# Deci-AI/super-gradients

Measured on NVIDIA H100. Metric: images/sec YOLO-NAS-S 640 bf16 train, higher is better.
Workload: dtype bf16

## Files before the change

### include/sgb200.h

```cpp
#ifndef SGB200_H_
#define SGB200_H_

#include <stdint.h>

#ifdef __cplusplus
extern "C" {
#endif

#define SGB_OK 0
#define SGB_E_INVALID (-1)
#define SGB_E_UNSUPPORTED (-2)
#define SGB_E_CUDA (-3)
#define SGB_E_ARCH (-4)

#define SGB_ACT_NONE 0
#define SGB_ACT_RELU 1
#define SGB_ACT_SILU 2

typedef uint16_t sgb_bf16;

typedef struct SgbConvDesc {
  int32_t N, H, W, C;
  int32_t K, R, S;
  int32_t P, Q;
  int32_t stride, pad;
  int32_t x_pitch, x_off;
  int32_t y_pitch, y_off;
  int32_t up2;
  int32_t centre_from;
} SgbConvDesc;

typedef struct SgbEpilogue {
  const float* scale;
  const float* shift;
  const sgb_bf16* residual;
  double* stats;
  int32_t stats_repl;
  int32_t act;
  int32_t out_f32;
} SgbEpilogue;

const char* sgb_last_error(void);
int sgb_version(void);
int sgb_check_device(void);
int64_t sgb_sm100_launches(void);
int64_t sgb_conv_halo_launches(void);
void sgb_conv_force_im2col(int on);
int64_t sgb_conv_wgrad_halo_launches(void);
void sgb_conv_wgrad_force_im2col(int on);

int sgb_conv_fprop(const SgbConvDesc* d, const sgb_bf16* x, const sgb_bf16* w_krsc, void* y, const SgbEpilogue* ep,
                   void* stream);
int sgb_conv_dgrad(const SgbConvDesc* d, const sgb_bf16* dy, const sgb_bf16* w_crsk, sgb_bf16* dx, int accumulate,
                   void* stream);
int sgb_conv_wgrad(const SgbConvDesc* d, const sgb_bf16* x, const sgb_bf16* dy, float* dw_krsc, void* stream);
int sgb_weight_prepare(const float* w_oihw, int K, int C, int R, int S, int c_pad, sgb_bf16* w_krsc, sgb_bf16* w_crsk,
                       const float* scale, int add_identity, void* stream);
int sgb_wgrad_to_oihw(const float* dw_krsc, int K, int C, int R, int S, int c_pad, float* g_oihw, int accumulate,
                      void* stream);
typedef struct SgbWeightItem {
  const float* w;
  const float* scale;
  sgb_bf16* krsc;
  sgb_bf16* crsk;
  int32_t K, C, R, S, c_pad, add_identity;
  int32_t kp, koff, etaps, etap;
  int64_t start;
} SgbWeightItem;
typedef struct SgbWgradItem {
  const float* dw;
  float* g;
  int32_t K, C, R, S, c_pad, accumulate;
  int64_t start;
} SgbWgradItem;
int sgb_weight_prepare_batch(const SgbWeightItem* items_dev, int n_items, int64_t total, void* stream);
typedef struct SgbAlphaItem {
  const float* dw1;
  const float* w1;
  const float* alpha;
  const float* dab;
  const float* bias1;
  float* g_w1;
  float* g_bias;
  float* g_alpha;
  int32_t K, C, c_pad, pad_;
} SgbAlphaItem;
int sgb_qarep_alpha_finish_batch(const SgbAlphaItem* items_dev, int n_items, void* stream);
int sgb_wgrad_to_oihw_batch(const SgbWgradItem* items_dev, int n_items, int64_t total, void* stream);
int sgb_convt2x2_fprop(const SgbConvDesc* d, const sgb_bf16* x_small, const sgb_bf16* w_up, const float* bias,
                       sgb_bf16* y_up, void* stream);

int sgb_nchw_f32_to_nhwc_bf16(const float* x, int N, int C, int H, int W, sgb_bf16* y, int y_pitch, int y_off, int c_out,
                              void* stream);
int sgb_stem_patches_f32(const float* x, int N, int C, int H, int W, int R, int stride, int pad, sgb_bf16* y, int P, int Q, int c_out,
                         void* stream);
int sgb_nhwc_bf16_to_nchw_f32(const sgb_bf16* x, int N, int C, int H, int W, int x_pitch, int x_off, float* y,
                              void* stream);

typedef struct SgbBnDesc {
  int64_t M;
  int32_t C;
  int32_t x_pitch, x_off;
  int32_t y_pitch, y_off;
  int32_t r_pitch, r_off;
  float eps, momentum;
  int32_t act;
  int32_t stats_repl;
  int32_t dy_pitch, dy_off;
  int64_t hw;
  const float* sample_scale;
  int32_t dy2_split, dy2_pitch, dy2_off, dy2_reserved;
  const void* dy2;
  const double* count;
  float param_scale;
  int32_t count_reserved;
} SgbBnDesc;
int sgb_bn_act_fwd(const SgbBnDesc* d, const sgb_bf16* x, const double* stats, const float* gamma, const float* beta,
                   float* running_mean, float* running_var, const sgb_bf16* residual, sgb_bf16* y, float* save_mean,
                   float* save_rstd, void* stream);
int sgb_bn_act_infer(const SgbBnDesc* d, const sgb_bf16* x, const float* gamma, const float* beta,
                     const float* running_mean, const float* running_var, const sgb_bf16* residual, sgb_bf16* y,
                     void* stream);
int sgb_bn_act_bwd_reduce(const SgbBnDesc* d, const sgb_bf16* dy, const sgb_bf16* x, const sgb_bf16* y, const float* gamma,
                          const float* beta, const float* save_mean, const float* save_rstd, double* sums, void* stream);
int sgb_bn_act_bwd_apply(const SgbBnDesc* d, const sgb_bf16* dy, const sgb_bf16* x, const sgb_bf16* y,
                         const float* gamma, const float* beta, const float* save_mean, const float* save_rstd,
                         const double* sums, sgb_bf16* dx, sgb_bf16* dresidual, float* dgamma, float* dbeta, void* stream);
int sgb_channel_stats(const sgb_bf16* x, int64_t M, int C, int pitch, int off, double* stats, void* stream);

typedef struct SgbQarepDesc {
  int64_t M;
  int32_t C;
  int32_t pitch3, off3, pitchu, offu, pitcho, offo;
  float eps3, eps_post, momentum;
  int32_t act;
  int32_t use_post_bn;
  int32_t pitchd, offd;
  int32_t pitchr, offr;
  const void* res;
  const float* res_alpha;
  const double* count;
  float param_scale;
  int32_t count_reserved;
} SgbQarepDesc;
int sgb_qarep_moments(const SgbQarepDesc* d, const sgb_bf16* y3, const sgb_bf16* u, double* moments, void* stream);
int sgb_qarep_fwd(const SgbQarepDesc* d, const sgb_bf16* y3, const sgb_bf16* u, const double* moments,
                  const float* gamma3, const float* beta3, const float* bias1_alpha, const float* gamma_p,
                  const float* beta_p, float* rm3, float* rv3, float* rm_p, float* rv_p, sgb_bf16* out, float* coef,
                  void* stream);
int sgb_qarep_fwd_fused(const SgbQarepDesc* d, const sgb_bf16* y3, const sgb_bf16* u, double* moments, const float* gamma3,
                        const float* beta3, const float* bias1_alpha, const float* gamma_p, const float* beta_p, float* rm3, float* rv3,
                        float* rm_p, float* rv_p, sgb_bf16* out, float* coef, void* stream);
int sgb_qarep_bwd_reduce(const SgbQarepDesc* d, const sgb_bf16* dout, const sgb_bf16* out, const sgb_bf16* y3,
                         const sgb_bf16* u, const float* coef, double* sums, void* stream);
int sgb_qarep_bwd_apply(const SgbQarepDesc* d, const sgb_bf16* dout, const sgb_bf16* out, const sgb_bf16* y3,
                        const sgb_bf16* u, const float* coef, const double* sums, const float* gamma3,
                        const float* gamma_p, sgb_bf16* dy3, sgb_bf16* du, float* dgamma3, float* dbeta3,
                        float* dbias1a, float* dgamma_p, float* dbeta_p, void* stream);
int sgb_bn_act_bwd_fused(const SgbBnDesc* d, const sgb_bf16* dy, const sgb_bf16* x, const sgb_bf16* y, const float* gamma,
                         const float* beta, const float* save_mean, const float* save_rstd, double* sums, sgb_bf16* dx,
                         sgb_bf16* dresidual, float* dgamma, float* dbeta, void* stream);
int sgb_bn_act_fwd_fused(const SgbBnDesc* d, const sgb_bf16* x, double* stats, const float* gamma, const float* beta,
                         float* running_mean, float* running_var, const sgb_bf16* residual, sgb_bf16* y, float* save_mean,
                         float* save_rstd, void* stream);
int sgb_qarep_bwd_fused(const SgbQarepDesc* d, const sgb_bf16* dout, const sgb_bf16* y3, const sgb_bf16* u, const float* coef,
                        double* sums, const float* gamma3, const float* gamma_p, sgb_bf16* dy3, sgb_bf16* du, float* dgamma3,
                        float* dbeta3, float* dbias1a, float* dgamma_p, float* dbeta_p, void* stream);

int sgb_stem_gemm(const SgbQarepDesc* d, const sgb_bf16* xp, const sgb_bf16* w, sgb_bf16* y, void* stream);
int sgb_stem_qarep_moments(const SgbQarepDesc* d, const sgb_bf16* xp, const sgb_bf16* w, double* moments, void* stream);
int sgb_stem_qarep_fwd(const SgbQarepDesc* d, const sgb_bf16* xp, const sgb_bf16* w, const double* moments, const float* gamma3,
                       const float* beta3, const float* bias1_alpha, const float* gamma_p, const float* beta_p, float* rm3, float* rv3,
                       float* rm_p, float* rv_p, sgb_bf16* out, float* coef, void* stream);
int sgb_stem_qarep_bwd_reduce(const SgbQarepDesc* d, const sgb_bf16* dout, const sgb_bf16* xp, const sgb_bf16* w, const float* coef,
                              double* sums, void* stream);
int sgb_stem_qarep_bwd_apply(const SgbQarepDesc* d, const sgb_bf16* dout, const sgb_bf16* xp, const sgb_bf16* w, const float* coef,
                             const double* sums, const float* gamma3, const float* gamma_p, sgb_bf16* dy3, sgb_bf16* du, float* dgamma3,
                             float* dbeta3, float* dbias1a, float* dgamma_p, float* dbeta_p, void* stream);
int64_t sgb_stem_recompute_launches(void);


int sgb_maxpool_fwd(const sgb_bf16* x, int N, int H, int W, int C, int x_pitch, int x_off, int k, int stride, int pad,
                    sgb_bf16* y, int P, int Q, int y_pitch, int y_off, uint8_t* idx, void* stream);
int sgb_maxpool_bwd(const sgb_bf16* dy, int N, int H, int W, int C, int k, int stride, int pad, int P, int Q,
                    int dy_pitch, int dy_off, const uint8_t* idx, float* dx_f32, void* stream);
int sgb_maxpool_bwd_bf16(const sgb_bf16* dy, int N, int H, int W, int C, int k, int stride, int pad, int P, int Q,
                         int dy_pitch, int dy_off, const uint8_t* idx, sgb_bf16* dx, int dx_pitch, void* stream);
int sgb_axpby(const sgb_bf16* x1, int p1, int o1, float a, const sgb_bf16* x2, int p2, int o2, float b, sgb_bf16* y,
              int py, int oy, int64_t M, int C, void* stream);
int sgb_scale_add(const sgb_bf16* x1, int p1, int o1, const float* a_dev, const sgb_bf16* x2, int p2, int o2, sgb_bf16* y,
                  int py, int oy, int64_t M, int C, void* stream);
int sgb_scale_add_dot(const sgb_bf16* x1, int p1, int o1, const float* a_dev, const sgb_bf16* x2, int p2, int o2, const sgb_bf16* xd, int pd,
                      int od, sgb_bf16* y, int py, int oy, int64_t M, int C, double* out_dot, void* stream);
int sgb_channel_dot(const sgb_bf16* a, int pa, int oa, const sgb_bf16* b, int pb, int ob, int64_t M, int C, double* out,
                    void* stream);
int sgb_f32_to_bf16(const float* x, sgb_bf16* y, int64_t n, void* stream);
int sgb_avgpool_fwd(const sgb_bf16* x, int N, int HW, int C, sgb_bf16* y, void* stream);
int sgb_avgpool_bwd(const sgb_bf16* dy, int N, int HW, int C, sgb_bf16* dx, void* stream);

int sgb_dfl_decode(const sgb_bf16* reg, int reg_pitch, const sgb_bf16* cls, int cls_pitch, int N, int Hf, int Wf,
                   int L, int anchor_base, int ncls, int reg_max, float stride, float cell_offset, float* pred_bboxes,
                   float* pred_scores, float* cls_logits, float* reg_distri, void* stream);

int sgb_pose_keypoint_decode(const sgb_bf16* pose, int pose_pitch, const sgb_bf16* logit, int logit_pitch, int logit_off, int N,
                             int Hf, int Wf, int L, int anchor_base, int J, float stride, float cell_offset,
                             float offset_multiplier, int compensate_grid_cell_offset, float* pose_coords, float* pose_scores,
                             float* pose_logits, void* stream);

typedef struct SgbLossDesc {
  int32_t B, L, ncls, reg_max;
  int32_t n_max;
  int32_t topk;
  float alpha, beta;
  float w_cls, w_iou, w_dfl;
  int32_t iou_type;
} SgbLossDesc;
int sgb_tal_assign(const SgbLossDesc* d, const float* cls_logits, const float* reg_distri, const float* anchor_points,
                   const float* stride_tensor, const float* gt_boxes, const int32_t* gt_labels, const uint8_t* gt_valid,
                   int32_t* assigned_label, float* assigned_box, float* assigned_score, double* sums, void* workspace,
                   int64_t workspace_bytes, void* stream);
int64_t sgb_tal_workspace_bytes(const SgbLossDesc* d);
int sgb_atss_assign(const SgbLossDesc* d, const float* reg_distri, const float* anchors, const float* anchor_points,
                    const float* stride_tensor, const int32_t* level_sizes, int32_t n_levels, const float* gt_boxes,
                    const int32_t* gt_labels, const uint8_t* gt_valid, int32_t* assigned_label, float* assigned_box,
                    float* assigned_score, double* sums, void* workspace, int64_t workspace_bytes, void* stream);
int64_t sgb_atss_workspace_bytes(const SgbLossDesc* d);
int sgb_dfl_iou_loss_fwd_bwd(const SgbLossDesc* d, const float* cls_logits, const float* reg_distri,
                             const float* anchor_points, const float* stride_tensor, const int32_t* assigned_label,
                             const float* assigned_box, const float* assigned_score, double* sums, float grad_scale,
                             float* grad_cls, float* grad_reg, void* stream);
int sgb_focal_cls_fwd_bwd(const SgbLossDesc* d, const float* cls_logits, const int32_t* assigned_label,
                          const float* assigned_score, double* sums, float grad_scale, float alpha, float* grad_cls,
                          void* stream);
int sgb_loss_finalize(const SgbLossDesc* d, const double* sums, float* loss_out, void* stream);
int sgb_head_grad_scatter(const float* grad, int gC, int N, int HW, int L, int anchor_base, sgb_bf16* dy, int pitch,
                          void* stream);

typedef struct SgbPoseLossDesc {
  int32_t B, L, J, reg_max;
  int32_t n_max;
  int32_t topk;
  float alpha, beta;
  float w_cls, w_iou, w_dfl, w_pose_cls, w_pose_reg;
  int32_t iou_type;
  int32_t cls_type;
  int32_t pose_cls_type;
  int32_t multiply_by_oks;
  int32_t rescale_with_score;
} SgbPoseLossDesc;
int64_t sgb_pose_tal_workspace_bytes(const SgbPoseLossDesc* d);
int sgb_pose_tal_assign(const SgbPoseLossDesc* d, const float* cls_logits, const float* reg_distri, const float* pose_coords,
                        const float* anchor_points, const float* stride_tensor, const float* gt_boxes, const float* gt_poses,
                        const uint8_t* gt_crowd, const uint8_t* gt_valid, const float* sigmas, int32_t* assigned_gt,
                        float* assigned_score, double* sums, void* workspace, int64_t workspace_bytes, void* stream);
int sgb_pose_loss_fwd_bwd(const SgbPoseLossDesc* d, const float* cls_logits, const float* reg_distri, const float* pose_coords,
                          const float* pose_logits, const float* anchor_points, const float* stride_tensor,
                          const float* gt_boxes, const float* gt_poses, const float* sigmas, const int32_t* assigned_gt,
                          const float* assigned_score, double* sums, float grad_scale, float* grad_cls, float* grad_reg,
                          float* grad_pose, float* grad_pose_logits, void* stream);
int sgb_pose_loss_finalize(const SgbPoseLossDesc* d, const double* sums, float* loss_out, void* stream);

typedef struct SgbNmsDesc {
  int32_t B, L, ncls;
  float score_thr;
  double iou_thr;
  int32_t top_k, max_out;
  int32_t multi_label;
  int32_t class_agnostic;
  int32_t thr_inclusive;
} SgbNmsDesc;
int64_t sgb_nms_workspace_bytes(const SgbNmsDesc* d);
int sgb_batched_nms(const SgbNmsDesc* d, const float* boxes, const float* scores, float* out, int32_t* out_idx,
                    int32_t* out_count, void* workspace, int64_t workspace_bytes, void* stream);

int sgb_sliding_window_gather(const sgb_bf16* canvas, int32_t B, int32_t H, int32_t W, int32_t pitch, const int32_t* tiles_host,
                              const int32_t* tiles, int32_t T, int32_t tile, sgb_bf16* out, void* stream);
int64_t sgb_sliding_window_merge_workspace_bytes(int32_t B, const int32_t* image_tiles_host, int32_t T, int32_t P, int32_t ncls);
int sgb_sliding_window_merge(const float* rows, const int32_t* counts, const int32_t* tiles, const int32_t* image_tiles_host,
                             const int32_t* image_tiles, int32_t B, int32_t T, int32_t P, int32_t ncls, double iou_thr, float* out,
                             int32_t* out_count, void* workspace, int64_t workspace_bytes, void* stream);
int32_t sgb_sliding_window_merge_launches(int32_t B, const int32_t* image_tiles_host, int32_t T, int32_t P);

#define SGB_MATCH_MAX_THRESHOLDS 32
typedef struct SgbMatchDesc {
  int32_t B;
  int32_t max_preds;
  int32_t max_targets;
  int32_t max_crowd;
  int32_t n_thresholds;
  int32_t top_k;
  int32_t denormalize_targets;
  float height, width;
} SgbMatchDesc;
int sgb_detection_matching(const SgbMatchDesc* d, const float* preds, const int32_t* pred_count, const float* targets,
                           const int32_t* target_count, const float* crowd, const int32_t* crowd_count, const float* thresholds,
                           uint8_t* matched, uint8_t* ignore, void* stream);

#define SGB_DISTANCE_EUCLIDEAN 0
#define SGB_DISTANCE_MANHATTAN 1
int sgb_detection_distance_matching(const SgbMatchDesc* d, int32_t metric, const float* preds, const int32_t* pred_count,
                                    const float* targets, const int32_t* target_count, const float* crowd,
                                    const int32_t* crowd_count, const float* thresholds, uint8_t* matched, uint8_t* ignore,
                                    void* stream);

int sgb_pose_keypoint_matching(const float* poses, const float* scores, const int32_t* pred_count, const float* gt_joints,
                               const float* gt_boxes, const float* gt_areas, const uint8_t* gt_flags, const int32_t* gt_count,
                               const float* sigmas, const float* thresholds, int32_t B, int32_t max_preds, int32_t max_targets,
                               int32_t n_joints, int32_t n_thresholds, int32_t top_k, uint8_t* matched, uint8_t* ignore,
                               float* used_scores, int32_t* used_count, int32_t* n_targets, float* oks_out, void* stream);

typedef struct SgbPreprocDesc {
  int32_t src_h, src_w, src_c;
  int32_t src_pitch;
  int32_t dst_h, dst_w;
  int32_t out_h, out_w;
  int32_t pad_top, pad_left;
  int32_t out_pitch;
  int32_t reverse_channels;
  int32_t normalize;
  float pad_value;
  double max_value;
  float mean[4], std[4];
} SgbPreprocDesc;
int sgb_preprocess_u8(const SgbPreprocDesc* d, const uint8_t* src, sgb_bf16* out, void* stream);

#define SGB_RS_OFFSET 0
#define SGB_RS_H 1
#define SGB_RS_W 2
#define SGB_RS_PITCH 3
#define SGB_RS_RESIZED_H 4
#define SGB_RS_RESIZED_W 5
#define SGB_RS_CROP_TOP 6
#define SGB_RS_CROP_LEFT 7
#define SGB_RS_FIELDS 8
int sgb_resample_crop_u8(const int64_t* table_host, const int64_t* table, const uint8_t* src, int64_t src_bytes, int32_t batch,
                         int32_t channels, int32_t out_h, int32_t out_w, int32_t out_pitch, int32_t reverse_channels,
                         double max_value, const float* mean_host, const float* std_host, sgb_bf16* out, void* stream);

#define SGB_AUG_OFFSET 0
#define SGB_AUG_H 1
#define SGB_AUG_W 2
#define SGB_AUG_AFFINE 3
#define SGB_AUG_AFF_H 4
#define SGB_AUG_AFF_W 5
#define SGB_AUG_M 6
#define SGB_AUG_AFF_BORDER 12
#define SGB_AUG_SWAP 13
#define SGB_AUG_HSV 14
#define SGB_AUG_DH 15
#define SGB_AUG_DS 16
#define SGB_AUG_DV 17
#define SGB_AUG_BGR 18
#define SGB_AUG_FLIP 19
#define SGB_AUG_MIX 20
#define SGB_AUG_MIX_OFFSET 21
#define SGB_AUG_MIX_H 22
#define SGB_AUG_MIX_W 23
#define SGB_AUG_MIX_FLIP 24
#define SGB_AUG_MIX_R1_H 25
#define SGB_AUG_MIX_R1_W 26
#define SGB_AUG_MIX_CANVAS_H 27
#define SGB_AUG_MIX_CANVAS_W 28
#define SGB_AUG_MIX_BORDER 29
#define SGB_AUG_MIX_R2_H 30
#define SGB_AUG_MIX_R2_W 31
#define SGB_AUG_MIX_X 32
#define SGB_AUG_MIX_Y 33
#define SGB_AUG_RS_H 34
#define SGB_AUG_RS_W 35
#define SGB_AUG_MOS 36
#define SGB_AUG_MOS_CANVAS_H 37
#define SGB_AUG_MOS_CANVAS_W 38
#define SGB_AUG_MOS_XC 39
#define SGB_AUG_MOS_YC 40
#define SGB_AUG_MOS_BORDER 41
#define SGB_AUG_MOS_TILE 42
#define SGB_AUG_MOS_TILES 4
#define SGB_AUG_T_OFFSET 0
#define SGB_AUG_T_H 1
#define SGB_AUG_T_W 2
#define SGB_AUG_T_RH 3
#define SGB_AUG_T_RW 4
#define SGB_AUG_T_X1 5
#define SGB_AUG_T_Y1 6
#define SGB_AUG_T_X2 7
#define SGB_AUG_T_Y2 8
#define SGB_AUG_T_SX 9
#define SGB_AUG_T_SY 10
#define SGB_AUG_MOS_TILE_FIELDS 11
#define SGB_AUG_FIELDS 86
int sgb_detection_augment(const int64_t* table_host, const int64_t* table, const uint8_t* src, int64_t src_bytes, int32_t batch,
                          int32_t channels, int32_t out_h, int32_t out_w, int32_t out_pitch, int32_t pad_value, double max_value,
                          int32_t hsv_simd_block, sgb_bf16* out, void* stream);

#define SGB_IN_OFFSET 0
#define SGB_IN_H 1
#define SGB_IN_W 2
#define SGB_IN_FILTER 3
#define SGB_IN_FLIP 4
#define SGB_IN_WS_OFFSET 5
#define SGB_IN_OP 6
#define SGB_IN_OP_FIELDS 7
#define SGB_IN_OPS 2
#define SGB_IN_FIELDS 20
#define SGB_IN_OP_NONE 0
#define SGB_IN_OP_AFFINE 1
#define SGB_IN_OP_INVERT 2
#define SGB_IN_OP_POSTERIZE 3
#define SGB_IN_OP_SOLARIZE 4
#define SGB_IN_OP_SOLARIZE_ADD 5
#define SGB_IN_OP_BRIGHTNESS 6
#define SGB_IN_OP_CONTRAST 7
#define SGB_IN_OP_AUTOCONTRAST 8
#define SGB_IN_OP_EQUALIZE 9
#define SGB_IN_OP_COLOR 10
#define SGB_IN_OP_SHARPNESS 11
int sgb_imagenet_augment(const int64_t* table_host, const int64_t* table, const uint8_t* src, int64_t src_bytes, uint8_t* workspace,
                         int64_t workspace_bytes, int32_t batch, int32_t size, int32_t out_pitch, const int32_t* fill_host,
                         const float* mean_host, const float* std_host, int32_t mix_mode, float lam, float one_minus_lam,
                         const int32_t* box_host, sgb_bf16* out, void* stream);

#define SGB_CF_SOURCE 0
#define SGB_CF_TOP 1
#define SGB_CF_LEFT 2
#define SGB_CF_FLIP 3
#define SGB_CF_FIELDS 4
#define SGB_CF_SIZE 32
#define SGB_CF_PAD 4
int sgb_cifar_augment(const int32_t* table_host, const int32_t* table, const uint8_t* src, int64_t src_images, int32_t batch,
                      int32_t out_pitch, const float* mean_host, const float* std_host, sgb_bf16* out, void* stream);

#define SGB_POSE_NSUB 0
#define SGB_POSE_CANVAS_H 1
#define SGB_POSE_CANVAS_W 2
#define SGB_POSE_MOSAIC_PAD 3
#define SGB_POSE_RS_H 4
#define SGB_POSE_RS_W 5
#define SGB_POSE_PAD_TOP 6
#define SGB_POSE_PAD_LEFT 7
#define SGB_POSE_PAD_VALUE 8
#define SGB_POSE_SUB 16
#define SGB_POSE_SUB_FIELDS 32
#define SGB_POSE_FIELDS 144
#define SGB_POSE_S_OFFSET 0
#define SGB_POSE_S_H 1
#define SGB_POSE_S_W 2
#define SGB_POSE_S_FLIP 3
#define SGB_POSE_S_BC 4
#define SGB_POSE_S_MEAN 5
#define SGB_POSE_S_CONTRAST 8
#define SGB_POSE_S_BRIGHTNESS 9
#define SGB_POSE_S_REVERSE 10
#define SGB_POSE_S_HSV 11
#define SGB_POSE_S_DH 12
#define SGB_POSE_S_DS 13
#define SGB_POSE_S_DV 14
#define SGB_POSE_S_ROT 15
#define SGB_POSE_S_AFFINE 16
#define SGB_POSE_S_M 17
#define SGB_POSE_S_MODE 23
#define SGB_POSE_S_BORDER 24
#define SGB_POSE_S_WS_OFFSET 25
#define SGB_POSE_S_Y 26
#define SGB_POSE_S_X 27
#define SGB_POSE_S_RH 28
#define SGB_POSE_S_RW 29
int sgb_pose_augment(const int64_t* table_host, const int64_t* table, const uint8_t* src, int64_t src_bytes, uint8_t* workspace,
                     int64_t workspace_bytes, int32_t batch, int32_t out_size, int32_t out_pitch, double max_value, int32_t hsv_simd_block,
                     sgb_bf16* out, void* stream);

int sgb_classify_rows(const void* logits, int64_t N, int32_t C, int64_t row_stride, int32_t logits_bf16, const int64_t* target,
                      const void* soft_target, int64_t target_stride, int32_t target_bf16, int32_t k, int64_t* counters,
                      int32_t* label, float* confidence, void* stream);

int sgb_sgd_step(float* p, const float* g, float* mom, int64_t n, const float* hp, void* stream);
int sgb_adamw_step(float* p, const float* g, float* m, float* v, int64_t n, const float* hp, void* stream);
int sgb_adam_step(float* p, const float* g, float* m, float* v, int64_t n, const float* hp, void* stream);
int sgb_rmsprop_step(float* p, const float* g, float* square_avg, float* momentum_buffer, float* grad_avg, int64_t n, const float* hp, void* stream);
int sgb_rmsprop_tf_step(float* p, const float* g, float* square_avg, float* momentum_buffer, float* grad_avg, int64_t n, const float* hp, void* stream);
int sgb_lion_step(float* p, const float* g, float* m, int64_t n, const float* hp, void* stream);
int sgb_lamb_grad_sqnorm(const float* g, const int64_t* chunks, int32_t nchunk, const float* hp, double* partials, void* stream);
int sgb_lamb_step(float* p, const float* g, float* m, float* v, float* update, int64_t n_decay, const int64_t* chunks, int32_t nchunk,
                  const float* hp, double* partials, void* stream);
int sgb_clip_grad_norm(const float* g, const int64_t* chunks, int32_t nchunk, float* hp, int32_t hp_len, int32_t gs_col, float max_norm, double* partials,
                       float* norm_coef, void* stream);
int sgb_ema_update(float* ema, const float* p, int64_t n, const float* decay, void* stream);

#define SGB_AVG_MAX_SLOTS 64
int sgb_average_snapshots(const float* const* slots, int32_t k, int64_t n, float* out, void* stream);

#ifdef __cplusplus
}
#endif
#endif
```

### super_gradients_b200/csrc/capi.cu

```cuda
#include <cstdarg>
#include <cstdio>

#include "common.cuh"
#include "conv_sm100.h"

static thread_local char g_err[512] = "";

void sgb_set_error(const char* fmt, ...) {
  va_list ap;
  va_start(ap, fmt);
  vsnprintf(g_err, sizeof(g_err), fmt, ap);
  va_end(ap);
}

int sgb_cuda_check(cudaError_t e, const char* what) {
  if (e == cudaSuccess) return SGB_OK;
  sgb_set_error("%s: %s", what, cudaGetErrorString(e));
  return SGB_E_CUDA;
}

extern "C" const char* sgb_last_error(void) { return g_err; }
extern "C" int sgb_version(void) { return 100; }
extern "C" int sgb_check_device(void) {
  int dev = 0;
  if (int rc = sgb_cuda_check(cudaGetDevice(&dev), "cudaGetDevice")) return rc;
  cudaDeviceProp prop;
  if (int rc = sgb_cuda_check(cudaGetDeviceProperties(&prop, dev), "cudaGetDeviceProperties")) return rc;
  if (prop.major != 9) {
    sgb_set_error("libsgb200 is built for sm_90a only; device is sm_%d%d", prop.major, prop.minor);
    return SGB_E_ARCH;
  }
  return SGB_OK;
}

extern "C" int64_t sgb_sm100_launches(void) { return (int64_t)sm100::launch_count(); }
extern "C" int64_t sgb_conv_halo_launches(void) { return (int64_t)sm100::halo_launch_count(); }
extern "C" void sgb_conv_force_im2col(int on) { sm100::force_im2col(on != 0); }
extern "C" int64_t sgb_conv_wgrad_halo_launches(void) { return (int64_t)sm100::wgrad_halo_launch_count(); }
extern "C" void sgb_conv_wgrad_force_im2col(int on) { sm100::wgrad_force_im2col(on != 0); }
```

### super_gradients_b200/csrc/conv_sm100.cu

```cuda
#include <cuda.h>

#include <cstdio>
#include <cstdlib>
#include <cstring>

#include "common.cuh"
#include "conv_sm100.h"
#include "sm100_host.h"
#include "sm100_ptx.cuh"

namespace sm100 {

constexpr int BLOCK_M = 128;
constexpr int NUM_THREADS = 384;
constexpr int CONSUMER_THREADS = 256;
constexpr int MAX_STAGES = 8;

struct Params {
  int M;
  int N;
  int C;
  int KC;
  int n_tiles;
  int stages;
  int P, Q;
  int stride, pad;
  int b_cols_per_tap;
  int ntaps;
  signed char tap_dh[9], tap_dw[9], tap_b[9];
  int out_mode, o_mul, oh_add, ow_add, outH, outW;
  int halo_tw, halo_thw;
  long long y_pitch;
  int y_off;
  bf16* y;
  const float* scale;
  const float* shift;
  const bf16* residual;
  double* stats;
  int stats_repl;
  int act;
  int centre_n, centre_c;
};

template <int BN>
__device__ __forceinline__ int off_centre_steps(const Params& p, int nt, int steps, int step_ch) {
  if (p.centre_n > 0 && nt * BN >= p.centre_n) return 0;
  if (p.centre_c > 0) return (p.centre_c + step_ch - 1) / step_ch;
  return steps;
}
constexpr int CENTRE_TAP = 4;

__device__ __forceinline__ long long out_row(const Params& p, long long m) {
  if (p.out_mode == 0) return m;
  const int pq = p.P * p.Q;
  const int n = (int)(m / pq);
  const int rem = (int)(m - (long long)n * pq);
  const int j = rem / p.Q, i = rem - j * p.Q;
  return ((long long)n * p.outH + j * p.o_mul + p.oh_add) * p.outW + i * p.o_mul + p.ow_add;
}

__device__ __forceinline__ void consumer_sync() { asm volatile("bar.sync 1, %0;" ::"n"(CONSUMER_THREADS) : "memory"); }
template <int WARPS>
__device__ __forceinline__ void group_sync(int wg) {
  if (WARPS == 8)
    consumer_sync();
  else
    asm volatile("bar.sync %0, 128;" ::"r"(2 + wg) : "memory");
}

constexpr uint32_t CTRL_BAR_BYTES = 16u * MAX_STAGES;

template <int BN, int WARPS = 8>
__device__ __forceinline__ void tile_epilogue(const Params& p, const float (&acc)[BN / 2], const long long (&orow)[2],
                                              const bool (&row_ok)[2], int nt, int wg, int wq, int lane, float* s_part,
                                              float* s_stats) {
  const int n0 = nt * BN;
  const int ncols = min(BN, p.N - n0);
  bf16* yrow[2];
  const bf16* rrow[2];
#pragma unroll
  for (int h = 0; h < 2; ++h) {
    yrow[h] = p.y + orow[h] * p.y_pitch + p.y_off + n0;
    rrow[h] = p.residual ? p.residual + orow[h] * p.y_pitch + p.y_off + n0 : nullptr;
  }
#pragma unroll
  for (int j = 0; j < BN / 8; ++j) {
    const int col = 8 * j + 2 * (lane & 3);
    const bool col_ok = col < ncols;
    float sum0 = 0.f, sum1 = 0.f, sq0 = 0.f, sq1 = 0.f;
#pragma unroll
    for (int h = 0; h < 2; ++h) {
      float v0 = acc[4 * j + 2 * h], v1 = acc[4 * j + 2 * h + 1];
      const bool ok = row_ok[h] && col_ok;
      if (p.scale && col_ok) {
        v0 *= p.scale[n0 + col];
        v1 *= p.scale[n0 + col + 1];
      }
      if (p.shift && col_ok) {
        v0 += p.shift[n0 + col];
        v1 += p.shift[n0 + col + 1];
      }
      if (rrow[h] && ok) {
        const uint32_t rr = *reinterpret_cast<const uint32_t*>(rrow[h] + col);
        v0 += __uint_as_float(rr << 16);
        v1 += __uint_as_float(rr & 0xffff0000u);
      }
      if (p.act != SGB_ACT_NONE) {
        v0 = apply_act(v0, p.act);
        v1 = apply_act(v1, p.act);
      }
      __nv_bfloat162 hh = __floats2bfloat162_rn(v0, v1);
      const uint32_t pk = *reinterpret_cast<uint32_t*>(&hh);
      if (ok) {
        *reinterpret_cast<uint32_t*>(yrow[h] + col) = pk;
        const float lo = __uint_as_float(pk << 16), hi = __uint_as_float(pk & 0xffff0000u);
        sum0 += lo;
        sum1 += hi;
        sq0 = fmaf(lo, lo, sq0);
        sq1 = fmaf(hi, hi, sq1);
      }
    }
    if (p.stats) {
#pragma unroll
      for (int o = 4; o < 32; o <<= 1) {
        sum0 += __shfl_xor_sync(0xffffffffu, sum0, o);
        sum1 += __shfl_xor_sync(0xffffffffu, sum1, o);
        sq0 += __shfl_xor_sync(0xffffffffu, sq0, o);
        sq1 += __shfl_xor_sync(0xffffffffu, sq1, o);
      }
      if (lane < 4) {
        float* part = s_part + (WARPS == 8 ? wg * 4 + wq : wq) * 2 * BN;
        part[col] = sum0;
        part[col + 1] = sum1;
        part[BN + col] = sq0;
        part[BN + col + 1] = sq1;
      }
    }
  }
  if (p.stats) {
    group_sync<WARPS>(wg);
    for (int i = threadIdx.x - 128 - (WARPS == 8 ? 0 : 128 * wg); i < 2 * BN; i += WARPS * 32) {
      const int which = i / BN, c = i - which * BN;
      if (c < ncols) {
        float v = 0.f;
#pragma unroll
        for (int w = 0; w < WARPS; ++w) v += s_part[w * 2 * BN + i];
        s_stats[which * p.N + n0 + c] += v;
      }
    }
    group_sync<WARPS>(wg);
  }
}

__device__ __forceinline__ void flush_stats(const Params& p, const float* s_stats) {
  if (p.stats) {
    double* st = p.stats + (long long)(blockIdx.x & (p.stats_repl - 1)) * 2 * p.N;
    for (int i = threadIdx.x; i < 2 * p.N; i += NUM_THREADS) {
      const float v = s_stats[i];
      if (v != 0.f) atomicAdd(&st[i], (double)v);
    }
  }
}

template <int BN, bool SKIP>
__global__ void __launch_bounds__(NUM_THREADS, 1)
conv_wgmma_kernel(const __grid_constant__ CUtensorMap map_a, const __grid_constant__ CUtensorMap map_b, const Params p) {
  extern __shared__ __align__(1024) unsigned char smem_raw[];
  const uint32_t smem_base = (smem_u32(smem_raw) + 1023u) & ~1023u;
  const uint32_t a_bytes = BLOCK_M * p.KC * 2, b_bytes = BN * p.KC * 2;
  const uint32_t stage_bytes = a_bytes + ((b_bytes + 1023u) & ~1023u);
  const uint32_t ctrl = smem_base + p.stages * stage_bytes;
  auto full_bar = [&](int s) { return ctrl + 8u * s; };
  auto empty_bar = [&](int s) { return ctrl + 8u * (MAX_STAGES + s); };
  float* s_part = reinterpret_cast<float*>(smem_raw + (ctrl + CTRL_BAR_BYTES - smem_u32(smem_raw)));
  float* s_stats = s_part + 8 * 2 * BN;

  const int warp = threadIdx.x >> 5, lane = threadIdx.x & 31;
  const int m_tiles = (p.M + BLOCK_M - 1) / BLOCK_M;
  const int total_tiles = m_tiles * p.n_tiles;
  const int chunks = (p.C + p.KC - 1) / p.KC;

  if (threadIdx.x == 0) {
    for (int s = 0; s < p.stages; ++s) {
      mbar_init(full_bar(s), 1);
      mbar_init(empty_bar(s), 8);
    }
    asm volatile("fence.mbarrier_init.release.cluster;" ::: "memory");
    asm volatile("fence.proxy.async.shared::cta;" ::: "memory");
  }
  if (p.stats)
    for (int i = threadIdx.x; i < 2 * p.N; i += NUM_THREADS) s_stats[i] = 0.f;
  __syncthreads();

  if (warp == 0) {
    if (elect_one()) {
      int stg = 0;
      uint32_t par = 1;
      const int pq = p.P * p.Q;
      for (int tile = blockIdx.x; tile < total_tiles; tile += gridDim.x) {
        const int mt = tile / p.n_tiles, nt = tile - mt * p.n_tiles;
        const int m0 = mt * BLOCK_M;
        const int n_img = m0 / pq;
        const int rem = m0 - n_img * pq;
        const int p0 = rem / p.Q, q0 = rem - p0 * p.Q;
        const int w0 = q0 * p.stride - p.pad, h0 = p0 * p.stride - p.pad;
        const int off = SKIP ? off_centre_steps<BN>(p, nt, chunks, p.KC) : chunks;
        for (int tap = 0; tap < p.ntaps; ++tap) {
          const int r = p.tap_dh[tap], s = p.tap_dw[tap];
          const int btap = p.tap_b[tap];
          const int n_ck = tap == CENTRE_TAP ? chunks : off;
          for (int ck = 0; ck < n_ck; ++ck) {
            mbar_wait(empty_bar(stg), par);
            const uint32_t sa = smem_base + stg * stage_bytes, sb = sa + a_bytes;
            mbar_expect_tx(full_bar(stg), a_bytes + b_bytes);
            tma_load_im2col_4d(sa, &map_a, full_bar(stg), ck * p.KC, w0, h0, n_img, (uint16_t)s, (uint16_t)r);
            tma_load_2d(sb, &map_b, full_bar(stg), btap * p.b_cols_per_tap + ck * p.KC, nt * BN);
            if (++stg == p.stages) {
              stg = 0;
              par ^= 1;
            }
          }
        }
      }
    }
  } else if (warp >= 4) {
    const int wg = (warp >> 2) - 1;
    const int wq = warp & 3;
    const int row_bytes = p.KC * 2;
    const uint32_t sbo = 8u * (uint32_t)row_bytes;
    const int ksteps = p.KC / 16;
    float acc[BN / 2];
    int stg = 0;
    uint32_t par = 0;
    for (int tile = blockIdx.x; tile < total_tiles; tile += gridDim.x) {
      const int mt = tile / p.n_tiles, nt = tile - mt * p.n_tiles;
      const int k_iters = SKIP ? 8 * off_centre_steps<BN>(p, nt, chunks, p.KC) + chunks : p.ntaps * chunks;
      int prev = -1;
      for (int k = 0; k < k_iters; ++k) {
        mbar_wait(full_bar(stg), par);
        const uint32_t sa = smem_base + stg * stage_bytes, sb = sa + a_bytes;
        const uint32_t sa_wg = sa + (uint32_t)wg * 64u * (uint32_t)row_bytes;
        wgmma_fence();
        for (int j = 0; j < ksteps; ++j) {
          const uint64_t da = smem_desc(sa_wg + 32u * j, row_bytes, 16u, sbo), db = smem_desc(sb + 32u * j, row_bytes, 16u, sbo);
          mma_kk<BN>(acc, da, db, (k | j) != 0);
        }
        wgmma_commit();
        if (prev >= 0) {
          wgmma_wait<1>();
          __syncwarp();
          if (lane == 0) mbar_arrive(empty_bar(prev));
        }
        prev = stg;
        if (++stg == p.stages) {
          stg = 0;
          par ^= 1;
        }
      }
      wgmma_wait<0>();
      fence_regs(acc);
      __syncwarp();
      if (lane == 0 && prev >= 0) mbar_arrive(empty_bar(prev));

      const long long m_lo = (long long)mt * BLOCK_M + wg * 64 + wq * 16 + (lane >> 2);
      long long orow[2];
      bool row_ok[2];
#pragma unroll
      for (int h = 0; h < 2; ++h) {
        const long long m = m_lo + 8 * h;
        row_ok[h] = m < p.M;
        orow[h] = out_row(p, row_ok[h] ? m : 0);
      }
      tile_epilogue<BN>(p, acc, orow, row_ok, nt, wg, wq, lane, s_part, s_stats);
    }
  }
  __syncthreads();
  flush_stats(p, s_stats);
}

constexpr int HALO_W = 10, HALO_H = 10, HALO_TILE = 8;
constexpr uint32_t HALO_CG_BYTES = 1664;
constexpr uint32_t HALO_CTRL_BYTES = CTRL_BAR_BYTES + 16;
constexpr int HALO_MAX_STAGES = 6;

template <int BN, bool SKIP>
__global__ void __launch_bounds__(NUM_THREADS, BN <= 48 ? 2 : 1)
conv3x3_halo_kernel(const __grid_constant__ CUtensorMap map_a, const __grid_constant__ CUtensorMap map_b, const Params p) {
  extern __shared__ __align__(1024) unsigned char smem_raw[];
  const uint32_t smem_base = (smem_u32(smem_raw) + 1023u) & ~1023u;
  const int ksteps = p.C / 16;
  constexpr uint32_t b_box = BN * 32;
  const uint32_t b_bytes = 9u * ksteps * b_box;
  const uint32_t a_stage = ((uint32_t)(p.C / 8) * HALO_CG_BYTES + 1023u) & ~1023u;
  const uint32_t sb = smem_base, sa0 = smem_base + ((b_bytes + 1023u) & ~1023u);
  const uint32_t ctrl = sa0 + p.stages * a_stage;
  auto full_bar = [&](int s) { return ctrl + 8u * s; };
  auto empty_bar = [&](int s) { return ctrl + 8u * (MAX_STAGES + s); };
  const uint32_t b_bar = ctrl + CTRL_BAR_BYTES;
  float* s_part = reinterpret_cast<float*>(smem_raw + (ctrl + HALO_CTRL_BYTES - smem_u32(smem_raw)));
  float* s_stats = s_part + 8 * 2 * BN;

  const int warp = threadIdx.x >> 5, lane = threadIdx.x & 31;
  const int m_tiles = p.M;
  const int nt = blockIdx.x % p.n_tiles;
  const int mt_step = gridDim.x / p.n_tiles;
  const int mt0 = blockIdx.x / p.n_tiles;
  const int off = SKIP ? off_centre_steps<BN>(p, nt, ksteps, 16) : ksteps;

  if (threadIdx.x == 0) {
    for (int s = 0; s < p.stages; ++s) {
      mbar_init(full_bar(s), 1);
      mbar_init(empty_bar(s), 4);
    }
    mbar_init(b_bar, 1);
    asm volatile("fence.mbarrier_init.release.cluster;" ::: "memory");
    asm volatile("fence.proxy.async.shared::cta;" ::: "memory");
  }
  if (p.stats)
    for (int i = threadIdx.x; i < 4 * p.N; i += NUM_THREADS) s_stats[i] = 0.f;
  __syncthreads();

  if (warp == 0) {
    if (elect_one()) {
      mbar_expect_tx(b_bar, (uint32_t)(8 * off + ksteps) * b_box);
      for (int bt = 0; bt < 9; ++bt)
        for (int ks = 0; ks < (bt == CENTRE_TAP ? ksteps : off); ++ks)
          tma_load_2d(sb + (uint32_t)(bt * ksteps + ks) * b_box, &map_b, b_bar, bt * p.b_cols_per_tap + 16 * ks, nt * BN);
      const uint32_t a_tx = (uint32_t)(p.C / 8) * (HALO_H * HALO_W * 16);
      int stg = 0;
      uint32_t par = 1;
      for (int mt = mt0; mt < m_tiles; mt += mt_step) {
        const int n_img = mt / p.halo_thw;
        const int rem = mt - n_img * p.halo_thw;
        const int th = rem / p.halo_tw, tw = rem - th * p.halo_tw;
        mbar_wait(empty_bar(stg), par);
        const uint32_t sa = sa0 + stg * a_stage;
        mbar_expect_tx(full_bar(stg), a_tx);
        for (int cg = 0; cg < p.C / 8; ++cg)
          tma_load_tiled_4d(sa + (uint32_t)cg * HALO_CG_BYTES, &map_a, full_bar(stg), 8 * cg, tw * HALO_TILE - 1, th * HALO_TILE - 1,
                            n_img);
        if (++stg == p.stages) {
          stg = 0;
          par ^= 1;
        }
      }
    }
  } else if (warp >= 4) {
    const int wg = (warp >> 2) - 1;
    const int wq = warp & 3;
    float acc[BN / 2];
    mbar_wait(b_bar, 0);
    for (int j = wg, mt = mt0 + wg * mt_step; mt < m_tiles; j += 2, mt += 2 * mt_step) {
      const int stg = j % p.stages;
      mbar_wait(full_bar(stg), (uint32_t)(j / p.stages) & 1u);
      const uint32_t sa = sa0 + stg * a_stage;
      wgmma_fence();
      int t = off > 0 ? 0 : CENTRE_TAP;
      uint32_t sa_t = sa + (uint32_t)((t / 3) * HALO_W + t % 3) * 16u, sb_t = sb + (uint32_t)(p.tap_b[t] * ksteps) * b_box;
      for (int k = 0, ks = 0, nk = 8 * off + ksteps; k < nk; ++k) {
        const uint64_t da = smem_desc_noswizzle(sa_t + (uint32_t)(2 * ks) * HALO_CG_BYTES, HALO_CG_BYTES, HALO_W * 16);
        const uint64_t db = smem_desc(sb_t + (uint32_t)ks * b_box, 32, 16u, 256u);
        mma_kk<BN>(acc, da, db, k != 0);
        if (++ks == (t == CENTRE_TAP ? ksteps : off) && ++t < 9) {
          ks = 0;
          sa_t = sa + (uint32_t)((t / 3) * HALO_W + t % 3) * 16u;
          sb_t = sb + (uint32_t)(p.tap_b[t] * ksteps) * b_box;
        }
      }
      wgmma_commit();
      wgmma_wait<0>();
      fence_regs(acc);
      __syncwarp();
      if (lane == 0) mbar_arrive(empty_bar(stg));

      const int n_img = mt / p.halo_thw;
      const int rem = mt - n_img * p.halo_thw;
      const int th = rem / p.halo_tw, tw = rem - th * p.halo_tw;
      const int ow = tw * HALO_TILE + (lane >> 2);
      long long orow[2];
      bool row_ok[2];
#pragma unroll
      for (int h = 0; h < 2; ++h) {
        const int oh = th * HALO_TILE + 2 * wq + h;
        row_ok[h] = oh < p.P && ow < p.Q;
        orow[h] = row_ok[h] ? ((long long)n_img * p.P + oh) * p.Q + ow : 0;
      }
      tile_epilogue<BN, 4>(p, acc, orow, row_ok, nt, wg, wq, lane, s_part + wg * 4 * 2 * BN, s_stats + wg * 2 * p.N);
    }
  }
  __syncthreads();
  if (p.stats) {
    for (int i = threadIdx.x; i < 2 * p.N; i += NUM_THREADS) s_stats[i] += s_stats[2 * p.N + i];
    __syncthreads();
  }
  flush_stats(p, s_stats);
}

struct WParams {
  int K, C;
  int R, S, stride, pad, P, Q;
  int npix;
  int CB;
  int n_ctiles;
  int rb_all, rb_off;
  int items;
  int pix_per_cta;
  int stages;
  int cpad;
  float* dw;
  int halo_tw, halo_thw, tiles, tiles_per_cta;
};
constexpr int WPIX = 64;

__host__ __device__ __forceinline__ int wgrad_row_blocks(const WParams& p, int tap) {
  return p.R * p.S == 9 && tap != CENTRE_TAP ? p.rb_off : p.rb_all;
}

template <int NB>
__global__ void __launch_bounds__(NUM_THREADS, 1)
wgrad_wgmma_kernel(const __grid_constant__ CUtensorMap map_dy, const __grid_constant__ CUtensorMap map_x, const WParams p) {
  extern __shared__ __align__(1024) unsigned char smem_raw[];
  const uint32_t smem_base = (smem_u32(smem_raw) + 1023u) & ~1023u;
  const uint32_t a_bytes = 2 * WPIX * 128;
  const uint32_t b_box = WPIX * p.CB * 2;
  const int boxes = NB / p.CB;
  const uint32_t stage_bytes = a_bytes + (uint32_t)boxes * b_box;
  const uint32_t ctrl = smem_base + p.stages * stage_bytes;
  auto full_bar = [&](int s) { return ctrl + 8u * s; };
  auto empty_bar = [&](int s) { return ctrl + 8u * (MAX_STAGES + s); };

  const int warp = threadIdx.x >> 5, lane = threadIdx.x & 31;
  int w = blockIdx.x;
  const int split = w / (p.items * p.n_ctiles);
  w -= split * p.items * p.n_ctiles;
  int tap = 0, tap_items = (wgrad_row_blocks(p, 0) + 1) / 2;
  while (w >= tap_items * p.n_ctiles) {
    w -= tap_items * p.n_ctiles;
    tap_items = (wgrad_row_blocks(p, ++tap) + 1) / 2;
  }
  const int ctile = w / tap_items, item = w - ctile * tap_items;
  const bool shared_rows = 2 * item + 1 == wgrad_row_blocks(p, tap);
  const int row0 = 128 * item;
  const int pix0 = split * p.pix_per_cta;
  const int pix1 = min(pix0 + p.pix_per_cta, p.npix);
  const int n_iters = (pix1 - pix0 + WPIX - 1) / WPIX;

  if (threadIdx.x == 0) {
    for (int s = 0; s < p.stages; ++s) {
      mbar_init(full_bar(s), 1);
      mbar_init(empty_bar(s), shared_rows ? 4 : 8);
    }
    asm volatile("fence.mbarrier_init.release.cluster;" ::: "memory");
    asm volatile("fence.proxy.async.shared::cta;" ::: "memory");
  }
  __syncthreads();

  if (n_iters > 0) {
    if (warp == 0) {
      if (elect_one()) {
        const int pq = p.P * p.Q;
        const int r = tap / p.S, s = tap - r * p.S;
        int stg = 0;
        uint32_t par = 1;
        for (int it = 0; it < n_iters; ++it) {
          mbar_wait(empty_bar(stg), par);
          const uint32_t sa = smem_base + stg * stage_bytes, sb = sa + a_bytes;
          mbar_expect_tx(full_bar(stg), (shared_rows ? a_bytes / 2 : a_bytes) + (uint32_t)boxes * b_box);
          const int pix = pix0 + it * WPIX;
          tma_load_2d(sa, &map_dy, full_bar(stg), row0, pix);
          if (!shared_rows) tma_load_2d(sa + WPIX * 128, &map_dy, full_bar(stg), row0 + 64, pix);
          const int n_img = pix / pq;
          const int rem = pix - n_img * pq;
          const int p0 = rem / p.Q, q0 = rem - p0 * p.Q;
          const int w0 = q0 * p.stride - p.pad, h0 = p0 * p.stride - p.pad;
          for (int bx = 0; bx < boxes; ++bx)
            tma_load_im2col_4d(sb + (uint32_t)bx * b_box, &map_x, full_bar(stg), ctile * NB + bx * p.CB, w0, h0, n_img, (uint16_t)s,
                               (uint16_t)r);
          if (++stg == p.stages) {
            stg = 0;
            par ^= 1;
          }
        }
      }
    } else if (warp >= 4) {
      const int wg = (warp >> 2) - 1, wq = warp & 3;
      const int b_row_bytes = p.CB * 2;
      float acc[NB / 2];
      const int it0 = shared_rows ? wg : 0, it_step = shared_rows ? 2 : 1;
      const uint32_t a_off = shared_rows ? 0u : (uint32_t)wg * (WPIX * 128);
      int stg = it0, prev = -1;
      uint32_t par = 0;
      for (int it = it0; it < n_iters; it += it_step) {
        mbar_wait(full_bar(stg), par);
        const uint32_t sa = smem_base + stg * stage_bytes + a_off, sb = smem_base + stg * stage_bytes + a_bytes;
        wgmma_fence();
#pragma unroll
        for (int j = 0; j < WPIX / 16; ++j) {
          const uint64_t da = smem_desc(sa + (uint32_t)j * 16u * 128u, 128, WPIX * 128, 8 * 128);
          const uint64_t db = smem_desc(sb + (uint32_t)j * 16u * (uint32_t)b_row_bytes, b_row_bytes, b_box, 8u * (uint32_t)b_row_bytes);
          mma_mn<NB>(acc, da, db, (it != it0 || j != 0) ? 1u : 0u);
        }
        wgmma_commit();
        if (prev >= 0) {
          wgmma_wait<1>();
          __syncwarp();
          if (lane == 0) mbar_arrive(empty_bar(prev));
        }
        prev = stg;
        if ((stg += it_step) >= p.stages) {
          stg -= p.stages;
          par ^= 1;
        }
      }
      if (prev < 0) return;
      wgmma_wait<0>();
      fence_regs(acc);
      const int row_len = p.R * p.S * p.cpad;
#pragma unroll
      for (int h = 0; h < 2; ++h) {
        const int ko = row0 + (shared_rows ? 0 : wg * 64) + wq * 16 + (lane >> 2) + 8 * h;
        if (ko < p.K) {
          float* drow = p.dw + (long long)ko * row_len + tap * p.cpad + ctile * NB + 2 * (lane & 3);
#pragma unroll
          for (int j = 0; j < NB / 8; ++j)
            asm volatile("red.global.add.v2.f32 [%0], {%1, %2};" ::"l"(drow + 8 * j), "f"(acc[4 * j + 2 * h]), "f"(acc[4 * j + 2 * h + 1])
                         : "memory");
        }
      }
    }
  }
}

constexpr uint32_t WH_A_BYTES = WPIX * 128;

__host__ __device__ constexpr uint32_t wgrad_halo_stage_bytes(int nb) {
  return (WH_A_BYTES + (uint32_t)(nb / 8) * HALO_CG_BYTES + 1023u) & ~1023u;
}

template <int NB, int NT>
__device__ __forceinline__ void wgrad_halo_consume(const WParams& p, uint32_t ring, uint32_t bars, int t0, int t1, int tap0, int rb,
                                                   int ctile) {
  constexpr uint32_t stage_bytes = wgrad_halo_stage_bytes(NB);
  const int wq = (threadIdx.x >> 5) & 3, lane = threadIdx.x & 31;
  auto full_bar = [&](int s) { return bars + 8u * s; };
  auto empty_bar = [&](int s) { return bars + 8u * (MAX_STAGES + s); };
  float acc[NT > 0 ? NT : 1][NB / 2];
  int stg = 0, prev = 0;
  uint32_t par = 0;
  for (int mt = t0; mt < t1; ++mt) {
    mbar_wait(full_bar(stg), par);
    if constexpr (NT > 0) {
      const uint32_t sa = ring + stg * stage_bytes, sx = sa + WH_A_BYTES;
      wgmma_fence();
#pragma unroll
      for (int t = 0; t < NT; ++t) {
        const int tap = tap0 + t;
        const uint32_t sx_t = sx + (uint32_t)((tap / 3) * HALO_W + tap % 3) * 16u;
#pragma unroll
        for (int j = 0; j < WPIX / 16; ++j) {
          const uint64_t da = smem_desc(sa + (uint32_t)j * 16u * 128u, 128, WPIX * 128, 8 * 128);
          const uint64_t db = smem_desc_noswizzle(sx_t + (uint32_t)j * 2u * HALO_W * 16u, HALO_W * 16, HALO_CG_BYTES);
          mma_mn<NB>(acc[t], da, db, (mt != t0 || j != 0) ? 1u : 0u);
        }
      }
      wgmma_commit();
      wgmma_wait<1>();
    }
    __syncwarp();
    if (lane == 0 && mt != t0) mbar_arrive(empty_bar(prev));
    prev = stg;
    if (++stg == p.stages) {
      stg = 0;
      par ^= 1;
    }
  }
  if constexpr (NT > 0) {
    wgmma_wait<0>();
#pragma unroll
    for (int t = 0; t < NT; ++t) fence_regs(acc[t]);
  }
  __syncwarp();
  if (lane == 0) mbar_arrive(empty_bar(prev));
  if constexpr (NT > 0) {
    const int row_len = 9 * p.cpad;
#pragma unroll
    for (int h = 0; h < 2; ++h) {
      const int ko = 64 * rb + wq * 16 + (lane >> 2) + 8 * h;
      if (ko < p.K) {
        float* drow = p.dw + (long long)ko * row_len + tap0 * p.cpad + ctile * NB + 2 * (lane & 3);
#pragma unroll
        for (int t = 0; t < NT; ++t)
#pragma unroll
          for (int j = 0; j < NB / 8; ++j)
            asm volatile("red.global.add.v2.f32 [%0], {%1, %2};" ::"l"(drow + t * p.cpad + 8 * j), "f"(acc[t][4 * j + 2 * h]),
                         "f"(acc[t][4 * j + 2 * h + 1])
                         : "memory");
      }
    }
  }
}

template <int NB>
__global__ void __launch_bounds__(NUM_THREADS, 1)
wgrad3x3_halo_kernel(const __grid_constant__ CUtensorMap map_dy, const __grid_constant__ CUtensorMap map_x, const WParams p) {
  extern __shared__ __align__(1024) unsigned char smem_raw[];
  const uint32_t smem_base = (smem_u32(smem_raw) + 1023u) & ~1023u;
  constexpr uint32_t a_bytes = WH_A_BYTES, stage_bytes = wgrad_halo_stage_bytes(NB);
  const uint32_t ctrl = smem_base + p.stages * stage_bytes;
  auto full_bar = [&](int s) { return ctrl + 8u * s; };
  auto empty_bar = [&](int s) { return ctrl + 8u * (MAX_STAGES + s); };

  const int warp = threadIdx.x >> 5;
  const int items = p.rb_all * p.n_ctiles;
  const int split = blockIdx.x / items, item = blockIdx.x - split * items;
  const int ctile = item / p.rb_all, rb = item - ctile * p.rb_all;
  const bool all_taps = rb < p.rb_off;
  const int t0 = split * p.tiles_per_cta, t1 = min(t0 + p.tiles_per_cta, p.tiles);

  if (threadIdx.x == 0) {
    for (int s = 0; s < p.stages; ++s) {
      mbar_init(full_bar(s), 1);
      mbar_init(empty_bar(s), 8);
    }
    asm volatile("fence.mbarrier_init.release.cluster;" ::: "memory");
    asm volatile("fence.proxy.async.shared::cta;" ::: "memory");
  }
  __syncthreads();

  if (warp == 0) {
    if (elect_one()) {
      const uint32_t tx = a_bytes + (NB / 8) * (HALO_H * HALO_W * 16);
      int stg = 0;
      uint32_t par = 1;
      for (int mt = t0; mt < t1; ++mt) {
        const int n_img = mt / p.halo_thw;
        const int rem = mt - n_img * p.halo_thw;
        const int th = rem / p.halo_tw, tw = rem - th * p.halo_tw;
        mbar_wait(empty_bar(stg), par);
        const uint32_t sa = smem_base + stg * stage_bytes;
        mbar_expect_tx(full_bar(stg), tx);
        tma_load_tiled_4d(sa, &map_dy, full_bar(stg), 64 * rb, tw * HALO_TILE, th * HALO_TILE, n_img);
        for (int cg = 0; cg < NB / 8; ++cg)
          tma_load_tiled_4d(sa + a_bytes + (uint32_t)cg * HALO_CG_BYTES, &map_x, full_bar(stg), ctile * NB + 8 * cg,
                            tw * HALO_TILE - 1, th * HALO_TILE - 1, n_img);
        if (++stg == p.stages) {
          stg = 0;
          par ^= 1;
        }
      }
    }
  } else if (warp >= 4) {
    const int wg = (warp >> 2) - 1;
    const uint32_t ring = smem_base, bars = ctrl;
    if (!all_taps && wg == 0)
      wgrad_halo_consume<NB, 1>(p, ring, bars, t0, t1, CENTRE_TAP, rb, ctile);
    else if (!all_taps)
      wgrad_halo_consume<NB, 0>(p, ring, bars, t0, t1, 0, rb, ctile);
    else if (wg == 0)
      wgrad_halo_consume<NB, 5>(p, ring, bars, t0, t1, 0, rb, ctile);
    else
      wgrad_halo_consume<NB, 4>(p, ring, bars, t0, t1, 5, rb, ctile);
  }
}

typedef CUresult (*EncodeTiledFn)(CUtensorMap*, CUtensorMapDataType, cuuint32_t, void*, const cuuint64_t*, const cuuint64_t*,
                                  const cuuint32_t*, const cuuint32_t*, CUtensorMapInterleave, CUtensorMapSwizzle,
                                  CUtensorMapL2promotion, CUtensorMapFloatOOBfill);
typedef CUresult (*EncodeIm2colFn)(CUtensorMap*, CUtensorMapDataType, cuuint32_t, void*, const cuuint64_t*, const cuuint64_t*,
                                   const int*, const int*, cuuint32_t, cuuint32_t, const cuuint32_t*, CUtensorMapInterleave,
                                   CUtensorMapSwizzle, CUtensorMapL2promotion, CUtensorMapFloatOOBfill);
EncodeTiledFn g_tiled = nullptr;
EncodeIm2colFn g_im2col = nullptr;
int g_num_sms = 0;
long long g_launches = 0;
long long g_halo_launches = 0;
long long g_wgrad_halo_launches = 0;
bool g_force_im2col = false;
bool g_wgrad_force_im2col = false;
long long launch_count() { return g_launches; }
long long halo_launch_count() { return g_halo_launches; }
long long wgrad_halo_launch_count() { return g_wgrad_halo_launches; }
void force_im2col(bool on) { g_force_im2col = on; }
void wgrad_force_im2col(bool on) { g_wgrad_force_im2col = on; }

int init_driver() {
  if (g_tiled && g_im2col) return SGB_OK;
  cudaDriverEntryPointQueryResult qres;
  void* fn = nullptr;
  if (cudaGetDriverEntryPoint("cuTensorMapEncodeTiled", &fn, cudaEnableDefault, &qres) != cudaSuccess || !fn) {
    sgb_set_error("cuTensorMapEncodeTiled entry point not found");
    return SGB_E_CUDA;
  }
  g_tiled = (EncodeTiledFn)fn;
  fn = nullptr;
  if (cudaGetDriverEntryPoint("cuTensorMapEncodeIm2col", &fn, cudaEnableDefault, &qres) != cudaSuccess || !fn) {
    sgb_set_error("cuTensorMapEncodeIm2col entry point not found");
    return SGB_E_CUDA;
  }
  g_im2col = (EncodeIm2colFn)fn;
  int dev = 0;
  cudaGetDevice(&dev);
  cudaDeviceGetAttribute(&g_num_sms, cudaDevAttrMultiProcessorCount, dev);
  return SGB_OK;
}

int encode_tiled(CUtensorMap* map, const void* ptr, int rank, const cuuint64_t* dims, const cuuint64_t* byte_strides,
                 const cuuint32_t* box, CUtensorMapSwizzle swizzle, const char* what) {
  const cuuint32_t elem_strides[5] = {1, 1, 1, 1, 1};
  const CUresult r = g_tiled(map, CU_TENSOR_MAP_DATA_TYPE_BFLOAT16, (cuuint32_t)rank, const_cast<void*>(ptr), dims, byte_strides, box,
                             elem_strides, CU_TENSOR_MAP_INTERLEAVE_NONE, swizzle, CU_TENSOR_MAP_L2_PROMOTION_L2_128B,
                             CU_TENSOR_MAP_FLOAT_OOB_FILL_NONE);
  if (r == CUDA_SUCCESS) return SGB_OK;
  char shape[256] = "";
  for (int i = 0, n = 0; i < rank && n < (int)sizeof(shape); ++i)
    n += snprintf(shape + n, sizeof(shape) - n, "%s%llu (box %u, stride %llu)", i ? ", " : "", (unsigned long long)dims[i],
                  (unsigned)box[i], i ? (unsigned long long)byte_strides[i - 1] : 2ull);
  sgb_set_error("cuTensorMapEncodeTiled(%s) failed with %d: dims %s", what, (int)r, shape);
  return SGB_E_CUDA;
}

namespace {

CUtensorMapSwizzle swizzle_for(int kc) {
  return kc == 64 ? CU_TENSOR_MAP_SWIZZLE_128B : (kc == 32 ? CU_TENSOR_MAP_SWIZZLE_64B : CU_TENSOR_MAP_SWIZZLE_32B);
}

int encode_im2col(CUtensorMap* map, const void* ptr, int N, int H, int W, int C, int pitch, int stride, const int (&lower)[2],
                  const int (&upper)[2], int channels, int pixels, const char* what) {
  const cuuint64_t dims[4] = {(cuuint64_t)C, (cuuint64_t)W, (cuuint64_t)H, (cuuint64_t)N};
  const cuuint64_t strides[3] = {(cuuint64_t)pitch * 2, (cuuint64_t)W * pitch * 2, (cuuint64_t)H * W * pitch * 2};
  const cuuint32_t estr[4] = {1, (cuuint32_t)stride, (cuuint32_t)stride, 1};
  const CUresult r = g_im2col(map, CU_TENSOR_MAP_DATA_TYPE_BFLOAT16, 4, const_cast<void*>(ptr), dims, strides, lower, upper,
                              (cuuint32_t)channels, (cuuint32_t)pixels, estr, CU_TENSOR_MAP_INTERLEAVE_NONE, swizzle_for(channels),
                              CU_TENSOR_MAP_L2_PROMOTION_L2_128B, CU_TENSOR_MAP_FLOAT_OOB_FILL_NONE);
  if (r == CUDA_SUCCESS) return SGB_OK;
  sgb_set_error("cuTensorMapEncodeIm2col(%s) failed with %d (C=%d W=%d H=%d N=%d pitch=%d lower=%d,%d upper=%d,%d stride=%d box=%d)", what,
                (int)r, C, W, H, N, pitch, lower[0], lower[1], upper[0], upper[1], stride, channels);
  return SGB_E_CUDA;
}

int encode_halo_map(CUtensorMap* map, const void* x, int N, int H, int W, int C, int pitch) {
  const cuuint64_t dims[4] = {(cuuint64_t)C, (cuuint64_t)W, (cuuint64_t)H, (cuuint64_t)N};
  const cuuint64_t strides[3] = {(cuuint64_t)pitch * 2, (cuuint64_t)W * pitch * 2, (cuuint64_t)H * W * pitch * 2};
  const cuuint32_t box[4] = {8, HALO_W, HALO_H, 1};
  return encode_tiled(map, x, 4, dims, strides, box, CU_TENSOR_MAP_SWIZZLE_NONE, "halo");
}

struct Problem {
  const void* a;
  int N, H, W, C, a_pitch;
  const void* b;
  int b_rows, b_cols, b_cols_per_tap;
  int R, S, stride, pad, P, Q, flip;
  int ntaps;
  int tap_dh[9], tap_dw[9], tap_b[9];
  int out_mode, o_mul, oh_add, ow_add, outH, outW;
  void* y;
  int y_pitch, y_off;
  const float* scale;
  const float* shift;
  const void* residual;
  double* stats;
  int stats_repl, act;
  int centre_from;
};

bool supported(const Problem& q) {
  if (q.C % 16 != 0 || q.b_rows % 8 != 0) return false;
  if (!((q.R == 1 && q.S == 1) || (q.R == 3 && q.S == 3))) return false;
  if (q.stride != 1 && q.stride != 2) return false;
  if (q.a_pitch % 8 != 0 || q.y_pitch % 8 != 0 || q.y_off % 8 != 0) return false;
  if (((uintptr_t)q.a & 15) || ((uintptr_t)q.b & 15) || ((uintptr_t)q.y & 15)) return false;
  if ((long long)q.N * q.P * q.Q >= (1ll << 31)) return false;
  if (q.b_rows > 4096) return false;
  return true;
}

template <class Fn>
struct Variant {
  int bn;
  Fn fn;
  int regs = 0;
  bool ready = false;
};
typedef void (*ConvFn)(const CUtensorMap, const CUtensorMap, const Params);
typedef void (*WgradFn)(const CUtensorMap, const CUtensorMap, const WParams);
template <bool SKIP>
Variant<ConvFn> g_conv[6] = {{16, conv_wgmma_kernel<16, SKIP>}, {32, conv_wgmma_kernel<32, SKIP>},
                             {48, conv_wgmma_kernel<48, SKIP>}, {64, conv_wgmma_kernel<64, SKIP>},
                             {96, conv_wgmma_kernel<96, SKIP>}, {128, conv_wgmma_kernel<128, SKIP>}};
template <bool SKIP>
Variant<ConvFn> g_halo[6] = {{16, conv3x3_halo_kernel<16, SKIP>}, {32, conv3x3_halo_kernel<32, SKIP>},
                             {48, conv3x3_halo_kernel<48, SKIP>}, {64, conv3x3_halo_kernel<64, SKIP>},
                             {96, conv3x3_halo_kernel<96, SKIP>}, {128, conv3x3_halo_kernel<128, SKIP>}};
Variant<WgradFn> g_wgrad[6] = {{16, wgrad_wgmma_kernel<16>}, {32, wgrad_wgmma_kernel<32>}, {48, wgrad_wgmma_kernel<48>},
                               {64, wgrad_wgmma_kernel<64>}, {96, wgrad_wgmma_kernel<96>}, {128, wgrad_wgmma_kernel<128>}};
Variant<WgradFn> g_wgrad_halo[3] = {{16, wgrad3x3_halo_kernel<16>}, {32, wgrad3x3_halo_kernel<32>}, {48, wgrad3x3_halo_kernel<48>}};

template <class Fn, int N>
int prepare(Variant<Fn> (&table)[N], int bn, const char* what, Variant<Fn>*& var) {
  for (auto& v : table)
    if (v.bn == bn) var = &v;
  if (var->ready) return SGB_OK;
  if (int rc = sgb_cuda_check(cudaFuncSetAttribute(var->fn, cudaFuncAttributeMaxDynamicSharedMemorySize, 227 * 1024), what)) return rc;
  cudaFuncAttributes fa{};
  if (int rc = sgb_cuda_check(cudaFuncGetAttributes(&fa, var->fn), what)) return rc;
  var->regs = fa.numRegs;
  var->ready = true;
  return SGB_OK;
}

int max_ctas_per_sm(int regs) {
  const int ctas = 65536 / (((regs + 7) / 8) * 8 * NUM_THREADS);
  return ctas > 2 ? 2 : (ctas < 1 ? 1 : ctas);
}

int pick_bn(int n) {
  for (int bn : {16, 32, 48, 64, 96, 128})
    if (n <= bn) return bn;
  int best = 128, best_waste = (n + 127) / 128 * 128 - n;
  for (int bn : {96, 64}) {
    const int waste = (n + bn - 1) / bn * bn - n;
    if (waste < best_waste) { best_waste = waste; best = bn; }
  }
  return best;
}

size_t halo_smem(int C, int bn, int n, bool stats, int stages) {
  const size_t b_bytes = ((size_t)9 * C * bn * 2 + 1023) & ~(size_t)1023;
  const size_t a_stage = ((size_t)(C / 8) * HALO_CG_BYTES + 1023) & ~(size_t)1023;
  return 1024 + b_bytes + (size_t)stages * a_stage + HALO_CTRL_BYTES + (stats ? (size_t)(8 * 2 * bn + 4 * n) * 4 : 0);
}

bool halo_tiles_fit(int P, int Q) {
  const long long covered = (long long)((P + 7) / 8) * 8 * ((Q + 7) / 8) * 8;
  return 20ll * P * Q >= 17 * covered;
}

int halo_bn(const Problem& q) {
  if (q.R != 3 || q.S != 3 || q.stride != 1 || q.pad != 1 || q.ntaps > 0 || q.out_mode != 0) return 0;
  if (q.P != q.H || q.Q != q.W) return 0;
  if (!halo_tiles_fit(q.P, q.Q)) return 0;
  const int n = q.b_rows, full = pick_bn(n);
  auto waste = [&](int bn) { return (n + bn - 1) / bn * bn - n; };
  for (int bn : {full, 96, 64})
    if (bn <= full && (bn == full || (q.C <= 96 && bn >= 64 && waste(bn) <= waste(full))) &&
        halo_smem(q.C, bn, n, q.stats != nullptr, 2) <= 227 * 1024)
      return bn;
  return 0;
}

int launch_halo(const Problem& q, const Params& p0, int bn, cudaStream_t st) {
  Params p = p0;
  p.n_tiles = (p.N + bn - 1) / bn;
  p.halo_tw = (q.Q + HALO_TILE - 1) / HALO_TILE;
  p.halo_thw = p.halo_tw * ((q.P + HALO_TILE - 1) / HALO_TILE);
  p.M = q.N * p.halo_thw;
  p.centre_n = 0;
  Variant<ConvFn>* var = nullptr;
  if (int rc = prepare(p.centre_c > 0 ? g_halo<true> : g_halo<false>, bn, "conv3x3_halo_kernel", var)) return rc;
  int ctas_per_sm = max_ctas_per_sm(var->regs);
  int stages = 0;
  for (;; --ctas_per_sm) {
    const size_t budget = (ctas_per_sm == 1 ? 227u : 227u / ctas_per_sm - 1u) * 1024u;
    for (stages = HALO_MAX_STAGES; stages >= 2 && halo_smem(q.C, bn, p.N, p.stats != nullptr, stages) > budget; --stages) {
    }
    if (stages >= 2 || ctas_per_sm == 1) break;
  }
  if (stages < 2) { sgb_set_error("conv3x3_halo: tile does not fit shared memory"); return SGB_E_UNSUPPORTED; }
  p.stages = stages;
  const size_t smem = halo_smem(q.C, bn, p.N, p.stats != nullptr, stages);

  alignas(64) CUtensorMap map_a, map_b;
  if (int rc = encode_halo_map(&map_a, q.a, q.N, q.H, q.W, q.C, q.a_pitch)) return rc;
  const cuuint64_t b_dims[2] = {(cuuint64_t)q.b_cols, (cuuint64_t)q.b_rows}, b_strides[1] = {(cuuint64_t)q.b_cols * 2};
  const cuuint32_t b_box[2] = {16, (cuuint32_t)bn};
  if (int rc = encode_tiled(&map_b, q.b, 2, b_dims, b_strides, b_box, CU_TENSOR_MAP_SWIZZLE_32B, "halo B")) return rc;
  int per_nt = g_num_sms * ctas_per_sm / p.n_tiles;
  if (per_nt > p.M) per_nt = p.M;
  if (per_nt < 1) per_nt = 1;
  var->fn<<<per_nt * p.n_tiles, NUM_THREADS, smem, st>>>(map_a, map_b, p);
  ++g_launches;
  ++g_halo_launches;
  return sgb_cuda_check(cudaGetLastError(), "conv3x3_halo_kernel");
}

int launch(const Problem& q, cudaStream_t st) {
  if (int rc = init_driver()) return rc;
  Params p{};
  p.M = q.N * q.P * q.Q;
  p.N = q.b_rows;
  p.C = q.C;
  p.KC = q.C % 64 == 0 ? 64 : (q.C % 32 == 0 ? 32 : 16);
  if (p.KC < 64 && q.C > 32) p.KC = 64;
  const int bn = pick_bn(p.N);
  p.n_tiles = (p.N + bn - 1) / bn;
  p.P = q.P; p.Q = q.Q; p.stride = q.stride; p.pad = q.pad;
  if (q.ntaps > 0) {
    p.ntaps = q.ntaps;
    for (int t = 0; t < q.ntaps; ++t) { p.tap_dh[t] = (signed char)q.tap_dh[t]; p.tap_dw[t] = (signed char)q.tap_dw[t]; p.tap_b[t] = (signed char)q.tap_b[t]; }
  } else {
    p.ntaps = q.R * q.S;
    for (int t = 0; t < p.ntaps; ++t) {
      p.tap_dh[t] = (signed char)(t / q.S);
      p.tap_dw[t] = (signed char)(t % q.S);
      p.tap_b[t] = (signed char)(q.flip ? (p.ntaps - 1 - t) : t);
    }
  }
  if (p.ntaps > 9) return SGB_E_UNSUPPORTED;
  p.out_mode = q.out_mode; p.o_mul = q.o_mul; p.oh_add = q.oh_add; p.ow_add = q.ow_add; p.outH = q.outH; p.outW = q.outW;
  p.b_cols_per_tap = q.b_cols_per_tap;
  p.y = (bf16*)q.y; p.y_pitch = q.y_pitch; p.y_off = q.y_off;
  p.scale = q.scale; p.shift = q.shift; p.residual = (const bf16*)q.residual;
  p.stats = q.stats; p.stats_repl = q.stats_repl > 0 ? q.stats_repl : 1; p.act = q.act;
  if (q.centre_from > 0) {
    if (q.R != 3 || q.S != 3 || q.stride != 1 || q.pad != 1 || q.ntaps > 0 || q.centre_from % 16 != 0 ||
        q.centre_from >= (q.flip ? q.C : q.b_rows))
      return SGB_E_INVALID;
    (q.flip ? p.centre_c : p.centre_n) = q.centre_from;
  }
  if (!g_force_im2col)
    if (const int hbn = halo_bn(q)) return launch_halo(q, p, hbn, st);
  Variant<ConvFn>* var = nullptr;
  if (int rc = prepare(p.centre_n > 0 || p.centre_c > 0 ? g_conv<true> : g_conv<false>, bn, "conv_wgmma_kernel", var)) return rc;
  const uint32_t a_bytes = BLOCK_M * p.KC * 2, b_bytes = ((uint32_t)(bn * p.KC * 2) + 1023u) & ~1023u;
  const uint32_t stage_bytes = a_bytes + b_bytes;
  const uint32_t ctrl_bytes = CTRL_BAR_BYTES + (p.stats ? (uint32_t)(8 * 2 * bn + 2 * p.N) * 4u : 0u);
  int ctas_per_sm = max_ctas_per_sm(var->regs);
  int stages = 0;
  for (;; --ctas_per_sm) {
    const uint32_t budget = (ctas_per_sm == 1 ? 226u : 227u / ctas_per_sm - 1u) * 1024u;
    stages = budget > ctrl_bytes + 1024 ? (int)((budget - ctrl_bytes - 1024) / stage_bytes) : 0;
    if (stages > MAX_STAGES) stages = MAX_STAGES;
    if (stages >= 4 || ctas_per_sm == 1) break;
  }
  if (stages < 2) { sgb_set_error("conv_wgmma: tile does not fit shared memory"); return SGB_E_UNSUPPORTED; }
  p.stages = stages;
  const size_t smem = 1024 + (size_t)stages * stage_bytes + ctrl_bytes;

  alignas(64) CUtensorMap map_a, map_b;
  int lower[2] = {-q.pad, -q.pad}, upper[2] = {q.pad - (q.S - 1), q.pad - (q.R - 1)};
  if (q.ntaps > 0) {
    lower[0] = lower[1] = 0;
    upper[0] = q.Q - q.W;
    upper[1] = q.P - q.H;
  }
  if (int rc = encode_im2col(&map_a, q.a, q.N, q.H, q.W, q.C, q.a_pitch, q.stride, lower, upper, p.KC, BLOCK_M, "A")) return rc;
  const cuuint64_t b_dims[2] = {(cuuint64_t)q.b_cols, (cuuint64_t)q.b_rows}, b_strides[1] = {(cuuint64_t)q.b_cols * 2};
  const cuuint32_t b_box[2] = {(cuuint32_t)p.KC, (cuuint32_t)bn};
  if (int rc = encode_tiled(&map_b, q.b, 2, b_dims, b_strides, b_box, swizzle_for(p.KC), "B")) return rc;
  const int m_tiles = (p.M + BLOCK_M - 1) / BLOCK_M;
  int grid = m_tiles * p.n_tiles;
  if (grid > g_num_sms * ctas_per_sm) grid = g_num_sms * ctas_per_sm;
  var->fn<<<grid, NUM_THREADS, smem, st>>>(map_a, map_b, p);
  ++g_launches;
  return sgb_cuda_check(cudaGetLastError(), "conv_wgmma_kernel");
}

struct WgradProblem {
  const void* x;
  const void* dy;
  int N, H, W, C, x_pitch;
  int K, y_pitch;
  int R, S, stride, pad, P, Q;
  float* dw;
  int centre_from;
};

bool wgrad_supported(const WgradProblem& q) {
  if (q.C % 16 != 0 || q.K % 8 != 0) return false;
  if (!((q.R == 1 && q.S == 1) || (q.R == 3 && q.S == 3))) return false;
  if (q.pad != q.R / 2 || (q.stride != 1 && q.stride != 2)) return false;
  if (q.x_pitch % 8 != 0 || q.y_pitch % 8 != 0) return false;
  if (((uintptr_t)q.x & 15) || ((uintptr_t)q.dy & 15)) return false;
  if ((long long)q.N * q.P * q.Q >= (1ll << 31)) return false;
  return true;
}

int wgrad_halo_nb(const WgradProblem& q) {
  if (q.R != 3 || q.S != 3 || q.stride != 1 || q.pad != 1 || q.P != q.H || q.Q != q.W) return 0;
  if (!halo_tiles_fit(q.P, q.Q)) return 0;
  return q.C % 32 == 0 ? 32 : (q.C % 48 == 0 ? 48 : 16);
}

int launch_wgrad_halo(const WgradProblem& q, const WParams& p0, int nb, cudaStream_t st) {
  WParams p = p0;
  p.n_ctiles = q.C / nb;
  p.halo_tw = (q.Q + HALO_TILE - 1) / HALO_TILE;
  p.halo_thw = p.halo_tw * ((q.P + HALO_TILE - 1) / HALO_TILE);
  p.tiles = q.N * p.halo_thw;
  Variant<WgradFn>* var = nullptr;
  if (int rc = prepare(g_wgrad_halo, nb, "wgrad3x3_halo_kernel", var)) return rc;
  const int ctas_per_sm = max_ctas_per_sm(var->regs);
  const uint32_t stage_bytes = wgrad_halo_stage_bytes(nb);
  const uint32_t budget = (ctas_per_sm == 1 ? 227u : 113u) * 1024u - 1024u - CTRL_BAR_BYTES;
  p.stages = (int)(budget / stage_bytes);
  if (p.stages > MAX_STAGES) p.stages = MAX_STAGES;
  const size_t smem = 1024 + (size_t)p.stages * stage_bytes + CTRL_BAR_BYTES;
  const int items = p.rb_all * p.n_ctiles;
  int splits = g_num_sms * ctas_per_sm / items;
  if (splits < 1) splits = 1;
  p.tiles_per_cta = (p.tiles + splits - 1) / splits;
  splits = (p.tiles + p.tiles_per_cta - 1) / p.tiles_per_cta;

  alignas(64) CUtensorMap map_dy, map_x;
  const cuuint64_t dy_dims[4] = {(cuuint64_t)q.K, (cuuint64_t)q.Q, (cuuint64_t)q.P, (cuuint64_t)q.N};
  const cuuint64_t dy_strides[3] = {(cuuint64_t)q.y_pitch * 2, (cuuint64_t)q.Q * q.y_pitch * 2, (cuuint64_t)q.P * q.Q * q.y_pitch * 2};
  const cuuint32_t dy_box[4] = {64, HALO_TILE, HALO_TILE, 1};
  if (int rc = encode_tiled(&map_dy, q.dy, 4, dy_dims, dy_strides, dy_box, CU_TENSOR_MAP_SWIZZLE_128B, "dy tile")) return rc;
  if (int rc = encode_halo_map(&map_x, q.x, q.N, q.H, q.W, q.C, q.x_pitch)) return rc;
  var->fn<<<splits * items, NUM_THREADS, smem, st>>>(map_dy, map_x, p);
  ++g_launches;
  ++g_wgrad_halo_launches;
  return sgb_cuda_check(cudaGetLastError(), "wgrad3x3_halo_kernel");
}

int wgrad_launch(const WgradProblem& q, cudaStream_t st) {
  if (int rc = init_driver()) return rc;
  WParams p{};
  p.K = q.K; p.C = q.C; p.R = q.R; p.S = q.S; p.stride = q.stride; p.pad = q.pad; p.P = q.P; p.Q = q.Q;
  p.npix = q.N * q.P * q.Q;
  int nb = 16;
  for (int cand : {128, 96, 64, 48, 32})
    if (q.C % cand == 0) { nb = cand; break; }
  p.CB = nb % 64 == 0 ? 64 : (nb % 32 == 0 ? 32 : 16);
  p.n_ctiles = q.C / nb;
  if (q.centre_from != 0 && (q.R != 3 || q.S != 3 || q.stride != 1 || q.pad != 1 || q.centre_from < 0 || q.centre_from >= q.K ||
                             q.centre_from % 16 != 0))
    return SGB_E_INVALID;
  p.rb_all = (q.K + 63) / 64;
  p.rb_off = q.centre_from > 0 ? (q.centre_from + 63) / 64 : p.rb_all;
  p.items = 0;
  for (int t = 0; t < q.R * q.S; ++t) p.items += (wgrad_row_blocks(p, t) + 1) / 2;
  p.cpad = q.C;
  p.dw = q.dw;
  if (!g_wgrad_force_im2col)
    if (const int nb = wgrad_halo_nb(q)) return launch_wgrad_halo(q, p, nb, st);
  Variant<WgradFn>* var = nullptr;
  if (int rc = prepare(g_wgrad, nb, "wgrad_wgmma_kernel", var)) return rc;
  const uint32_t stage_bytes = 2 * WPIX * 128 + (uint32_t)(nb / p.CB) * WPIX * p.CB * 2;
  int stages = (int)((200 * 1024 - CTRL_BAR_BYTES - 1024) / stage_bytes);
  if (stages > MAX_STAGES) stages = MAX_STAGES;
  if (p.rb_all % 2 || p.rb_off % 2) stages &= ~1;
  if (stages < 2) return SGB_E_UNSUPPORTED;
  p.stages = stages;
  const size_t smem = 1024 + (size_t)stages * stage_bytes + CTRL_BAR_BYTES;
  const int base_ctas = p.items * p.n_ctiles;
  const int total_iters = (p.npix + WPIX - 1) / WPIX;
  int splits = (2 * g_num_sms + base_ctas - 1) / base_ctas;
  if (splits > total_iters / 8) splits = total_iters / 8;
  if (splits < 1) splits = 1;
  int iters_per = (total_iters + splits - 1) / splits;
  p.pix_per_cta = iters_per * WPIX;
  splits = (p.npix + p.pix_per_cta - 1) / p.pix_per_cta;

  alignas(64) CUtensorMap map_dy, map_x;
  const cuuint64_t dy_dims[2] = {(cuuint64_t)q.K, (cuuint64_t)p.npix}, dy_strides[1] = {(cuuint64_t)q.y_pitch * 2};
  const cuuint32_t dy_box[2] = {64, (cuuint32_t)WPIX};
  if (int rc = encode_tiled(&map_dy, q.dy, 2, dy_dims, dy_strides, dy_box, CU_TENSOR_MAP_SWIZZLE_128B, "dy")) return rc;
  const int lower[2] = {-q.pad, -q.pad}, upper[2] = {q.pad - (q.S - 1), q.pad - (q.R - 1)};
  if (int rc = encode_im2col(&map_x, q.x, q.N, q.H, q.W, q.C, q.x_pitch, q.stride, lower, upper, p.CB, WPIX, "x, wgrad")) return rc;
  const int grid = base_ctas * splits;
  var->fn<<<grid, NUM_THREADS, smem, st>>>(map_dy, map_x, p);
  ++g_launches;
  return sgb_cuda_check(cudaGetLastError(), "wgrad_wgmma_kernel");
}

Problem gemm(const sgb_bf16* a, int N, int H, int W, int C, int a_pitch, const sgb_bf16* b, int b_rows, int b_cols_per_tap, int R,
             int S, int stride, int pad, int P, int Q, void* y, int y_pitch, int y_off) {
  Problem q{};
  q.a = a; q.N = N; q.H = H; q.W = W; q.C = C; q.a_pitch = a_pitch;
  q.b = b; q.b_rows = b_rows; q.b_cols = R * S * b_cols_per_tap; q.b_cols_per_tap = b_cols_per_tap;
  q.R = R; q.S = S; q.stride = stride; q.pad = pad; q.P = P; q.Q = Q;
  q.y = y; q.y_pitch = y_pitch; q.y_off = y_off;
  q.stats_repl = 1;
  return q;
}

void parity_output(Problem& q, int ph, int pw, int outH, int outW) {
  q.out_mode = 1; q.o_mul = 2; q.oh_add = ph; q.ow_add = pw; q.outH = outH; q.outW = outW;
}

void stride2_taps(Problem& q, int ph, int pw, int pad) {
  q.ntaps = 0;
  for (int r = 0; r < q.R; ++r) {
    if (((ph + pad - r) & 1) != 0) continue;
    for (int s = 0; s < q.S; ++s) {
      if (((pw + pad - s) & 1) != 0) continue;
      q.tap_dh[q.ntaps] = (ph + pad - r) / 2;
      q.tap_dw[q.ntaps] = (pw + pad - s) / 2;
      q.tap_b[q.ntaps] = r * q.S + s;
      ++q.ntaps;
    }
  }
}

bool row_pairs(const SgbConvDesc& d, SgbConvDesc* pairs) {
  if (!(d.R == 2 && d.S == 2 && d.stride == 2 && d.pad == 0 && d.x_pitch == d.C && d.x_off == 0 && d.H % 2 == 0 && d.W % 2 == 0 &&
        d.P == d.H / 2 && d.Q == d.W / 2 && (2 * d.C) % 16 == 0 && d.K % 8 == 0 && d.y_pitch % 8 == 0 && d.y_off % 8 == 0 &&
        (long long)d.N * (d.H / 2) < (1ll << 31)))
    return false;
  *pairs = d;
  pairs->N = d.N * (d.H / 2); pairs->H = 2; pairs->W = d.W / 2; pairs->C = 2 * d.C; pairs->x_pitch = 2 * d.C;
  pairs->S = 1; pairs->stride = 1; pairs->P = 1; pairs->Q = d.W / 2;
  return true;
}

Problem fprop_problem(const SgbConvDesc& d, const sgb_bf16* x, const sgb_bf16* w, void* y, const SgbEpilogue* ep) {
  Problem q = gemm(x + d.x_off, d.N, d.H, d.W, d.C, d.x_pitch, w, d.K, d.C, d.R, d.S, d.stride, d.pad, d.P, d.Q, y, d.y_pitch, d.y_off);
  q.centre_from = d.centre_from;
  if (ep) {
    q.scale = ep->scale; q.shift = ep->shift; q.residual = ep->residual; q.stats = ep->stats;
    q.stats_repl = ep->stats_repl > 0 ? ep->stats_repl : 1; q.act = ep->act;
  }
  return q;
}

WgradProblem wgrad_problem(const SgbConvDesc& d, const sgb_bf16* x, const sgb_bf16* dy, float* dw) {
  WgradProblem q{};
  q.x = x + d.x_off; q.dy = dy + d.y_off;
  q.N = d.N; q.H = d.H; q.W = d.W; q.C = d.C; q.x_pitch = d.x_pitch;
  q.K = d.K; q.y_pitch = d.y_pitch;
  q.R = d.R; q.S = d.S; q.stride = d.stride; q.pad = d.pad; q.P = d.P; q.Q = d.Q;
  q.dw = dw;
  q.centre_from = d.centre_from;
  return q;
}

}

int conv_fprop(const SgbConvDesc& d, const sgb_bf16* x, const sgb_bf16* w, void* y, const SgbEpilogue* ep, cudaStream_t st) {
  if (ep && ep->out_f32) return DECLINED;
  if (d.pad == d.R / 2) {
    const Problem q = fprop_problem(d, x, w, y, ep);
    if (supported(q)) return launch(q, st);
  }
  SgbConvDesc pairs;
  if (!row_pairs(d, &pairs)) return DECLINED;
  Problem q = fprop_problem(pairs, x, w, y, ep);
  q.R = 1;
  q.ntaps = 2;
  q.tap_dh[1] = 1;
  q.tap_b[1] = 1;
  return supported(q) ? launch(q, st) : SGB_E_UNSUPPORTED;
}

int convt2x2_fprop(const SgbConvDesc& d, const sgb_bf16* x_small, const sgb_bf16* w_up, const float* bias, sgb_bf16* y_up,
                   cudaStream_t st) {
  if (d.K % 16 != 0 || d.C % 16 != 0) return DECLINED;
  for (int cls = 0; cls < 4; ++cls) {
    Problem q = gemm(x_small + d.y_off, d.N, d.P, d.Q, d.K, d.y_pitch, w_up + (size_t)cls * d.C * d.K, d.C, d.K, 1, 1, 1, 0, d.P,
                     d.Q, y_up, d.x_pitch, d.x_off);
    q.shift = bias;
    parity_output(q, cls >> 1, cls & 1, d.H, d.W);
    if (!supported(q)) return DECLINED;
    if (int rc = launch(q, st)) return rc;
  }
  return SGB_OK;
}

int conv_dgrad(const SgbConvDesc& d, const sgb_bf16* dy, const sgb_bf16* w_crsk, sgb_bf16* dx, int accumulate, cudaStream_t st) {
  const int Kp = ((d.K + 7) / 8) * 8;
  auto dgrad_gemm = [&](int pad, int P, int Q) {
    Problem q = gemm(dy + d.y_off, d.N, d.P, d.Q, d.K, d.y_pitch, w_crsk, d.C, Kp, d.R, d.S, 1, pad, P, Q, dx, d.x_pitch, d.x_off);
    q.residual = accumulate ? dx : nullptr;
    return q;
  };
  if (d.stride == 1 && d.pad == d.R / 2 && d.K % 16 == 0) {
    Problem q = dgrad_gemm(d.R - 1 - d.pad, d.H, d.W);
    q.flip = 1;
    q.centre_from = d.centre_from;
    if (supported(q)) return launch(q, st);
  }
  if (d.stride == 2 && d.K % 16 == 0 && d.R == 3 && d.S == 3 && d.pad == 1 && d.H == 2 * d.P && d.W == 2 * d.Q) {
    for (int cls = 0; cls < 4; ++cls) {
      Problem q = dgrad_gemm(0, d.P, d.Q);
      parity_output(q, cls >> 1, cls & 1, d.H, d.W);
      stride2_taps(q, cls >> 1, cls & 1, d.pad);
      if (!supported(q)) return DECLINED;
      if (int rc = launch(q, st)) return rc;
    }
    return SGB_OK;
  }
  if (d.stride == 2 && d.K % 16 == 0 && d.R == 1 && d.S == 1 && d.pad == 0 && d.H == 2 * d.P && d.W == 2 * d.Q) {
    Problem q = dgrad_gemm(0, d.P, d.Q);
    parity_output(q, 0, 0, d.H, d.W);
    const bool dense = d.x_pitch == d.C && d.x_off == 0;
    if (supported(q) && (accumulate || dense)) {
      if (!accumulate) cudaMemsetAsync(dx, 0, (size_t)d.N * d.H * d.W * d.C * sizeof(sgb_bf16), st);
      return launch(q, st);
    }
  }
  return DECLINED;
}

int conv_wgrad(const SgbConvDesc& d, const sgb_bf16* x, const sgb_bf16* dy, float* dw, cudaStream_t st) {
  const WgradProblem q = wgrad_problem(d, x, dy, dw);
  if (wgrad_supported(q)) return wgrad_launch(q, st);
  SgbConvDesc pairs;
  if (row_pairs(d, &pairs)) return wgrad_launch(wgrad_problem(pairs, x, dy, dw), st);
  return DECLINED;
}

}
```

### super_gradients_b200/csrc/conv_sm100.h

```cpp
#pragma once
#include <cuda_runtime.h>

#include "sgb200.h"

namespace sm100 {

constexpr int DECLINED = 1;

int conv_fprop(const SgbConvDesc& d, const sgb_bf16* x, const sgb_bf16* w, void* y, const SgbEpilogue* ep, cudaStream_t st);
int convt2x2_fprop(const SgbConvDesc& d, const sgb_bf16* x_small, const sgb_bf16* w_up, const float* bias, sgb_bf16* y_up,
                   cudaStream_t st);
int conv_dgrad(const SgbConvDesc& d, const sgb_bf16* dy, const sgb_bf16* w_crsk, sgb_bf16* dx, int accumulate, cudaStream_t st);
int conv_wgrad(const SgbConvDesc& d, const sgb_bf16* x, const sgb_bf16* dy, float* dw, cudaStream_t st);

long long launch_count();
long long halo_launch_count();
void force_im2col(bool on);
long long wgrad_halo_launch_count();
void wgrad_force_im2col(bool on);

}
```

### super_gradients_b200/csrc/sm100_host.h

```cpp
#pragma once

#include <cuda.h>

namespace sm100 {

int init_driver();

int encode_tiled(CUtensorMap* map, const void* ptr, int rank, const cuuint64_t* dims, const cuuint64_t* byte_strides,
                 const cuuint32_t* box, CUtensorMapSwizzle swizzle, const char* what);

}
```

### super_gradients_b200/lib.py

```python
import ctypes
import os
from ctypes import POINTER, Structure, c_char_p, c_double, c_float, c_int, c_int32, c_int64, c_void_p

_HERE = os.path.dirname(os.path.abspath(__file__))
LIB_PATH = os.path.join(_HERE, "libsgb200.so")

ACT_NONE, ACT_RELU, ACT_SILU = 0, 1, 2


class SgbError(RuntimeError):
    pass


class ConvDesc(Structure):
    _fields_ = [(n, c_int32) for n in ("N", "H", "W", "C", "K", "R", "S", "P", "Q", "stride", "pad", "x_pitch", "x_off", "y_pitch", "y_off", "up2", "centre_from")]


class Epilogue(Structure):
    _fields_ = [
        ("scale", c_void_p),
        ("shift", c_void_p),
        ("residual", c_void_p),
        ("stats", c_void_p),
        ("stats_repl", c_int32),
        ("act", c_int32),
        ("out_f32", c_int32),
    ]


class WeightItem(Structure):
    _fields_ = [("w", c_void_p), ("scale", c_void_p), ("krsc", c_void_p), ("crsk", c_void_p)] + [(n, c_int32) for n in ("K", "C", "R", "S", "c_pad", "add_identity", "kp", "koff", "etaps", "etap")] + [("start", c_int64)]


class WgradItem(Structure):
    _fields_ = [("dw", c_void_p), ("g", c_void_p)] + [(n, c_int32) for n in ("K", "C", "R", "S", "c_pad", "accumulate")] + [("start", c_int64)]


class AlphaItem(Structure):
    _fields_ = [(n, c_void_p) for n in ("dw1", "w1", "alpha", "dab", "bias1", "g_w1", "g_bias", "g_alpha")] + [(n, c_int32) for n in ("K", "C", "c_pad", "pad_")]


class BnDesc(Structure):
    _fields_ = [
        ("M", c_int64),
        ("C", c_int32),
        ("x_pitch", c_int32),
        ("x_off", c_int32),
        ("y_pitch", c_int32),
        ("y_off", c_int32),
        ("r_pitch", c_int32),
        ("r_off", c_int32),
        ("eps", c_float),
        ("momentum", c_float),
        ("act", c_int32),
        ("stats_repl", c_int32),
        ("dy_pitch", c_int32),
        ("dy_off", c_int32),
        ("hw", c_int64),
        ("sample_scale", c_void_p),
        ("dy2_split", c_int32),
        ("dy2_pitch", c_int32),
        ("dy2_off", c_int32),
        ("dy2_reserved", c_int32),
        ("dy2", c_void_p),
        ("count", c_void_p),
        ("param_scale", c_float),
        ("count_reserved", c_int32),
    ]


class QarepDesc(Structure):
    _fields_ = [
        ("M", c_int64),
        ("C", c_int32),
        ("pitch3", c_int32),
        ("off3", c_int32),
        ("pitchu", c_int32),
        ("offu", c_int32),
        ("pitcho", c_int32),
        ("offo", c_int32),
        ("eps3", c_float),
        ("eps_post", c_float),
        ("momentum", c_float),
        ("act", c_int32),
        ("use_post_bn", c_int32),
        ("pitchd", c_int32),
        ("offd", c_int32),
        ("pitchr", c_int32),
        ("offr", c_int32),
        ("res", c_void_p),
        ("res_alpha", c_void_p),
        ("count", c_void_p),
        ("param_scale", c_float),
        ("count_reserved", c_int32),
    ]


class PoseLossDesc(Structure):
    _fields_ = (
        [(n, c_int32) for n in ("B", "L", "J", "reg_max", "n_max", "topk")]
        + [(n, c_float) for n in ("alpha", "beta", "w_cls", "w_iou", "w_dfl", "w_pose_cls", "w_pose_reg")]
        + [(n, c_int32) for n in ("iou_type", "cls_type", "pose_cls_type", "multiply_by_oks", "rescale_with_score")]
    )


class PreprocDesc(Structure):
    _fields_ = (
        [(n, c_int32) for n in ("src_h", "src_w", "src_c", "src_pitch", "dst_h", "dst_w", "out_h", "out_w", "pad_top", "pad_left", "out_pitch", "reverse_channels", "normalize")]
        + [("pad_value", c_float), ("max_value", c_double), ("mean", c_float * 4), ("std", c_float * 4)]
    )


class MatchDesc(Structure):
    _fields_ = [(n, c_int32) for n in ("B", "max_preds", "max_targets", "max_crowd", "n_thresholds", "top_k", "denormalize_targets")] + [("height", c_float), ("width", c_float)]


class LossDesc(Structure):
    _fields_ = [
        ("B", c_int32),
        ("L", c_int32),
        ("ncls", c_int32),
        ("reg_max", c_int32),
        ("n_max", c_int32),
        ("topk", c_int32),
        ("alpha", c_float),
        ("beta", c_float),
        ("w_cls", c_float),
        ("w_iou", c_float),
        ("w_dfl", c_float),
        ("iou_type", c_int32),
    ]


class NmsDesc(Structure):
    _fields_ = [
        ("B", c_int32),
        ("L", c_int32),
        ("ncls", c_int32),
        ("score_thr", c_float),
        ("iou_thr", c_double),
        ("top_k", c_int32),
        ("max_out", c_int32),
        ("multi_label", c_int32),
        ("class_agnostic", c_int32),
        ("thr_inclusive", c_int32),
    ]


P = c_void_p
_I, _F, _L = c_int, c_float, c_int64

_SIGNATURES = {
    "sgb_last_error": (c_char_p, []),
    "sgb_version": (c_int, []),
    "sgb_check_device": (c_int, []),
    "sgb_sm100_launches": (c_int64, []),
    "sgb_conv_halo_launches": (c_int64, []),
    "sgb_conv_force_im2col": (None, [_I]),
    "sgb_conv_wgrad_halo_launches": (c_int64, []),
    "sgb_conv_wgrad_force_im2col": (None, [_I]),
    "sgb_conv_fprop": (c_int, [POINTER(ConvDesc), P, P, P, POINTER(Epilogue), P]),
    "sgb_conv_dgrad": (c_int, [POINTER(ConvDesc), P, P, P, _I, P]),
    "sgb_conv_wgrad": (c_int, [POINTER(ConvDesc), P, P, P, P]),
    "sgb_weight_prepare": (c_int, [P, _I, _I, _I, _I, _I, P, P, P, _I, P]),
    "sgb_wgrad_to_oihw": (c_int, [P, _I, _I, _I, _I, _I, P, _I, P]),
    "sgb_weight_prepare_batch": (c_int, [P, _I, c_int64, P]),
    "sgb_wgrad_to_oihw_batch": (c_int, [P, _I, c_int64, P]),
    "sgb_qarep_alpha_finish_batch": (c_int, [P, _I, P]),
    "sgb_convt2x2_fprop": (c_int, [POINTER(ConvDesc), P, P, P, P, P]),
    "sgb_nchw_f32_to_nhwc_bf16": (c_int, [P, _I, _I, _I, _I, P, _I, _I, _I, P]),
    "sgb_stem_patches_f32": (c_int, [P, _I, _I, _I, _I, _I, _I, _I, P, _I, _I, _I, P]),
    "sgb_nhwc_bf16_to_nchw_f32": (c_int, [P, _I, _I, _I, _I, _I, _I, P, P]),
    "sgb_bn_act_fwd": (c_int, [POINTER(BnDesc), P, P, P, P, P, P, P, P, P, P, P]),
    "sgb_bn_act_fwd_fused": (c_int, [POINTER(BnDesc), P, P, P, P, P, P, P, P, P, P, P]),
    "sgb_bn_act_infer": (c_int, [POINTER(BnDesc), P, P, P, P, P, P, P, P]),
    "sgb_bn_act_bwd_reduce": (c_int, [POINTER(BnDesc), P, P, P, P, P, P, P, P, P]),
    "sgb_bn_act_bwd_apply": (c_int, [POINTER(BnDesc), P, P, P, P, P, P, P, P, P, P, P, P, P]),
    "sgb_bn_act_bwd_fused": (c_int, [POINTER(BnDesc), P, P, P, P, P, P, P, P, P, P, P, P, P]),
    "sgb_channel_stats": (c_int, [P, _L, _I, _I, _I, P, P]),
    "sgb_qarep_moments": (c_int, [POINTER(QarepDesc), P, P, P, P]),
    "sgb_qarep_fwd": (c_int, [POINTER(QarepDesc)] + [P] * 15),
    "sgb_qarep_fwd_fused": (c_int, [POINTER(QarepDesc)] + [P] * 15),
    "sgb_qarep_bwd_reduce": (c_int, [POINTER(QarepDesc), P, P, P, P, P, P, P]),
    "sgb_qarep_bwd_apply": (c_int, [POINTER(QarepDesc)] + [P] * 16),
    "sgb_qarep_bwd_fused": (c_int, [POINTER(QarepDesc)] + [P] * 15),
    "sgb_stem_gemm": (c_int, [POINTER(QarepDesc), P, P, P, P]),
    "sgb_stem_qarep_moments": (c_int, [POINTER(QarepDesc), P, P, P, P]),
    "sgb_stem_qarep_fwd": (c_int, [POINTER(QarepDesc)] + [P] * 15),
    "sgb_stem_qarep_bwd_reduce": (c_int, [POINTER(QarepDesc)] + [P] * 6),
    "sgb_stem_qarep_bwd_apply": (c_int, [POINTER(QarepDesc)] + [P] * 15),
    "sgb_stem_recompute_launches": (c_int64, []),
    "sgb_maxpool_fwd": (c_int, [P, _I, _I, _I, _I, _I, _I, _I, _I, _I, P, _I, _I, _I, _I, P, P]),
    "sgb_maxpool_bwd": (c_int, [P, _I, _I, _I, _I, _I, _I, _I, _I, _I, _I, _I, P, P, P]),
    "sgb_maxpool_bwd_bf16": (c_int, [P, _I, _I, _I, _I, _I, _I, _I, _I, _I, _I, _I, P, P, _I, P]),
    "sgb_axpby": (c_int, [P, _I, _I, _F, P, _I, _I, _F, P, _I, _I, _L, _I, P]),
    "sgb_scale_add": (c_int, [P, _I, _I, P, P, _I, _I, P, _I, _I, _L, _I, P]),
    "sgb_channel_dot": (c_int, [P, _I, _I, P, _I, _I, _L, _I, P, P]),
    "sgb_scale_add_dot": (c_int, [P, _I, _I, P, P, _I, _I, P, _I, _I, P, _I, _I, _L, _I, P, P]),
    "sgb_f32_to_bf16": (c_int, [P, P, _L, P]),
    "sgb_avgpool_fwd": (c_int, [P, _I, _I, _I, P, P]),
    "sgb_avgpool_bwd": (c_int, [P, _I, _I, _I, P, P]),
    "sgb_dfl_decode": (c_int, [P, _I, P, _I, _I, _I, _I, _I, _I, _I, _I, _F, _F, P, P, P, P, P]),
    "sgb_pose_keypoint_decode": (c_int, [P, _I, P, _I, _I, _I, _I, _I, _I, _I, _I, _F, _F, _F, _I, P, P, P, P]),
    "sgb_tal_assign": (c_int, [POINTER(LossDesc)] + [P] * 12 + [_L, P]),
    "sgb_tal_workspace_bytes": (c_int64, [POINTER(LossDesc)]),
    "sgb_atss_assign": (c_int, [POINTER(LossDesc)] + [P] * 5 + [c_int32] + [P] * 7 + [P, _L, P]),
    "sgb_atss_workspace_bytes": (c_int64, [POINTER(LossDesc)]),
    "sgb_dfl_iou_loss_fwd_bwd": (c_int, [POINTER(LossDesc)] + [P] * 8 + [_F, P, P, P]),
    "sgb_focal_cls_fwd_bwd": (c_int, [POINTER(LossDesc), P, P, P, P, c_float, c_float, P, P]),
    "sgb_loss_finalize": (c_int, [POINTER(LossDesc), P, P, P]),
    "sgb_preprocess_u8": (c_int, [POINTER(PreprocDesc), P, P, P]),
    "sgb_resample_crop_u8": (c_int, [P, P, P, _L, _I, _I, _I, _I, _I, _I, c_double, P, P, P, P]),
    "sgb_classify_rows": (c_int, [P, _L, _I, _L, _I, P, P, _L, _I, _I, P, P, P, P]),
    "sgb_detection_augment": (c_int, [P, P, P, _L, _I, _I, _I, _I, _I, _I, c_double, _I, P, P]),
    "sgb_pose_augment": (c_int, [P, P, P, _L, P, _L, _I, _I, _I, c_double, _I, P, P]),
    "sgb_imagenet_augment": (c_int, [P, P, P, _L, P, _L, _I, _I, _I, P, P, P, _I, c_float, c_float, P, P, P]),
    "sgb_cifar_augment": (c_int, [P, P, P, _L, _I, _I, P, P, P, P]),
    "sgb_detection_matching": (c_int, [POINTER(MatchDesc), P, P, P, P, P, P, P, P, P, P]),
    "sgb_detection_distance_matching": (c_int, [POINTER(MatchDesc), c_int32, P, P, P, P, P, P, P, P, P, P]),
    "sgb_pose_keypoint_matching": (c_int, [P] * 10 + [_I] * 6 + [P] * 7),
    "sgb_pose_tal_workspace_bytes": (c_int64, [POINTER(PoseLossDesc)]),
    "sgb_pose_tal_assign": (c_int, [POINTER(PoseLossDesc)] + [P] * 14 + [_L, P]),
    "sgb_pose_loss_fwd_bwd": (c_int, [POINTER(PoseLossDesc)] + [P] * 12 + [_F] + [P] * 5),
    "sgb_pose_loss_finalize": (c_int, [POINTER(PoseLossDesc), P, P, P]),
    "sgb_head_grad_scatter": (c_int, [P, _I, _I, _I, _I, _I, P, _I, P]),
    "sgb_sliding_window_gather": (c_int, [P, _I, _I, _I, _I, P, P, _I, _I, P, P]),
    "sgb_sliding_window_merge_workspace_bytes": (c_int64, [_I, P, _I, _I, _I]),
    "sgb_sliding_window_merge": (c_int, [P, P, P, P, P, _I, _I, _I, _I, c_double, P, P, P, _L, P]),
    "sgb_sliding_window_merge_launches": (c_int32, [_I, P, _I, _I]),
    "sgb_nms_workspace_bytes": (c_int64, [POINTER(NmsDesc)]),
    "sgb_batched_nms": (c_int, [POINTER(NmsDesc), P, P, P, P, P, P, _L, P]),
    "sgb_sgd_step": (c_int, [P, P, P, _L, P, P]),
    "sgb_adamw_step": (c_int, [P, P, P, P, _L, P, P]),
    "sgb_ema_update": (c_int, [P, P, _L, P, P]),
    "sgb_adam_step": (c_int, [P, P, P, P, _L, P, P]),
    "sgb_rmsprop_step": (c_int, [P, P, P, P, P, _L, P, P]),
    "sgb_rmsprop_tf_step": (c_int, [P, P, P, P, P, _L, P, P]),
    "sgb_lion_step": (c_int, [P, P, P, _L, P, P]),
    "sgb_lamb_grad_sqnorm": (c_int, [P, P, c_int32, P, P, P]),
    "sgb_lamb_step": (c_int, [P, P, P, P, P, _L, P, c_int32, P, P, P]),
    "sgb_clip_grad_norm": (c_int, [P, P, c_int32, P, c_int32, c_int32, _F, P, P, P]),
    "sgb_average_snapshots": (c_int, [P, c_int32, _L, P, P]),
}

_lib = None

LAUNCH_COUNT = {"sgb_tal_assign": 4, "sgb_lamb_step": 2, "sgb_clip_grad_norm": 2, "sgb_atss_assign": 3, "sgb_pose_tal_assign": 4, "sgb_sm100_launches": 0, "sgb_stem_recompute_launches": 0, "sgb_conv_halo_launches": 0, "sgb_conv_force_im2col": 0, "sgb_conv_wgrad_halo_launches": 0, "sgb_conv_wgrad_force_im2col": 0, "sgb_sliding_window_merge_workspace_bytes": 0, "sgb_sliding_window_merge_launches": 0, "sgb_last_error": 0, "sgb_version": 0, "sgb_check_device": 0}
LAUNCHES = [0]


def exported_names():
    return sorted(_SIGNATURES)


def load():
    global _lib
    if _lib is not None:
        return _lib
    if not os.path.exists(LIB_PATH):
        raise SgbError(f"{LIB_PATH} not found: run `python -c 'import __graft_entry__ as g; g.build()'` " "(there is no non-CUDA fallback for this package)")
    lib = ctypes.CDLL(LIB_PATH)
    for name, (res, args) in _SIGNATURES.items():
        fn = getattr(lib, name)
        fn.restype = res
        fn.argtypes = args
    _lib = lib
    return lib


def check(rc, what=""):
    if rc != 0:
        msg = load().sgb_last_error()
        raise SgbError(f"{what} failed with code {rc}: {msg.decode() if msg else ''}")


def call(name, *args):
    lib = load()
    rc = getattr(lib, name)(*args)
    LAUNCHES[0] += LAUNCH_COUNT.get(name, 1)
    if rc != 0:
        msg = lib.sgb_last_error()
        raise SgbError(f"{name} failed with code {rc}: {msg.decode() if msg else ''}")
```

Measured before the change: 987.0.

## Add stride-2 halo TMA path for 3x3 conv fprop and wgrad

Extends the halo-tile 3x3 conv and wgrad kernels to stride 2. The input is loaded as four phase-split sub-tiles through TMA with element strides of 2, so each tap reads a contiguous 9x9 window instead of going through the im2col path. It is gated to small channel counts (C<=48) and large spatial sizes, which is where YOLO-NAS downsampling convs land. It also keeps KC at 32 for stride-2 dgrad with C=96. The cost is more template variants, an even stage count, and a larger shared-memory footprint per stage.

```diff
diff --git a/include/sgb200.h b/include/sgb200.h
--- a/include/sgb200.h
+++ b/include/sgb200.h
@@ -45,8 +45,10 @@
 int sgb_check_device(void);
 int64_t sgb_sm100_launches(void);
 int64_t sgb_conv_halo_launches(void);
+int64_t sgb_conv_halo_s2_launches(void);
 void sgb_conv_force_im2col(int on);
 int64_t sgb_conv_wgrad_halo_launches(void);
+int64_t sgb_conv_wgrad_halo_s2_launches(void);
 void sgb_conv_wgrad_force_im2col(int on);
 
 int sgb_conv_fprop(const SgbConvDesc* d, const sgb_bf16* x, const sgb_bf16* w_krsc, void* y, const SgbEpilogue* ep,
diff --git a/super_gradients_b200/csrc/capi.cu b/super_gradients_b200/csrc/capi.cu
--- a/super_gradients_b200/csrc/capi.cu
+++ b/super_gradients_b200/csrc/capi.cu
@@ -35,6 +35,8 @@
 
 extern "C" int64_t sgb_sm100_launches(void) { return (int64_t)sm100::launch_count(); }
 extern "C" int64_t sgb_conv_halo_launches(void) { return (int64_t)sm100::halo_launch_count(); }
+extern "C" int64_t sgb_conv_halo_s2_launches(void) { return (int64_t)sm100::halo_s2_launch_count(); }
 extern "C" void sgb_conv_force_im2col(int on) { sm100::force_im2col(on != 0); }
 extern "C" int64_t sgb_conv_wgrad_halo_launches(void) { return (int64_t)sm100::wgrad_halo_launch_count(); }
+extern "C" int64_t sgb_conv_wgrad_halo_s2_launches(void) { return (int64_t)sm100::wgrad_halo_s2_launch_count(); }
 extern "C" void sgb_conv_wgrad_force_im2col(int on) { sm100::wgrad_force_im2col(on != 0); }
diff --git a/super_gradients_b200/csrc/conv_sm100.cu b/super_gradients_b200/csrc/conv_sm100.cu
--- a/super_gradients_b200/csrc/conv_sm100.cu
+++ b/super_gradients_b200/csrc/conv_sm100.cu
@@ -280,18 +280,32 @@
 
 constexpr int HALO_W = 10, HALO_H = 10, HALO_TILE = 8;
 constexpr uint32_t HALO_CG_BYTES = 1664;
+constexpr int HALO_S2_W = 9;
+constexpr uint32_t HALO_S2_CG_BYTES = 1408;
 constexpr uint32_t HALO_CTRL_BYTES = CTRL_BAR_BYTES + 16;
 constexpr int HALO_MAX_STAGES = 6;
 
-template <int BN, bool SKIP>
+__host__ __device__ constexpr uint32_t halo_a_stage(int C, int stride) {
+  return ((uint32_t)(C / 8) * (stride == 1 ? HALO_CG_BYTES : 4u * HALO_S2_CG_BYTES) + 1023u) & ~1023u;
+}
+
+template <int BN, bool SKIP, int STRIDE>
 __global__ void __launch_bounds__(NUM_THREADS, BN <= 48 ? 2 : 1)
 conv3x3_halo_kernel(const __grid_constant__ CUtensorMap map_a, const __grid_constant__ CUtensorMap map_b, const Params p) {
+  static_assert(STRIDE == 1 || !SKIP, "zero taps are skipped at stride 1 only");
   extern __shared__ __align__(1024) unsigned char smem_raw[];
   const uint32_t smem_base = (smem_u32(smem_raw) + 1023u) & ~1023u;
   const int ksteps = p.C / 16;
   constexpr uint32_t b_box = BN * 32;
   const uint32_t b_bytes = 9u * ksteps * b_box;
-  const uint32_t a_stage = ((uint32_t)(p.C / 8) * HALO_CG_BYTES + 1023u) & ~1023u;
+  const uint32_t a_stage = halo_a_stage(p.C, STRIDE);
+  constexpr uint32_t a_cg = STRIDE == 1 ? HALO_CG_BYTES : HALO_S2_CG_BYTES, a_row = (STRIDE == 1 ? HALO_W : HALO_S2_W) * 16;
+  const uint32_t a_sub = (uint32_t)(p.C / 8) * HALO_S2_CG_BYTES;
+  auto a_tap = [&](int t) -> uint32_t {
+    const int dh = t / 3, dw = t % 3;
+    if (STRIDE == 1) return (uint32_t)(dh * HALO_W + dw) * 16u;
+    return (uint32_t)(2 * (dh == 1) + (dw == 1)) * a_sub + (uint32_t)((dh >> 1) * HALO_S2_W + (dw >> 1)) * 16u;
+  };
   const uint32_t sb = smem_base, sa0 = smem_base + ((b_bytes + 1023u) & ~1023u);
   const uint32_t ctrl = sa0 + p.stages * a_stage;
   auto full_bar = [&](int s) { return ctrl + 8u * s; };
@@ -326,7 +340,7 @@
       for (int bt = 0; bt < 9; ++bt)
         for (int ks = 0; ks < (bt == CENTRE_TAP ? ksteps : off); ++ks)
           tma_load_2d(sb + (uint32_t)(bt * ksteps + ks) * b_box, &map_b, b_bar, bt * p.b_cols_per_tap + 16 * ks, nt * BN);
-      const uint32_t a_tx = (uint32_t)(p.C / 8) * (HALO_H * HALO_W * 16);
+      const uint32_t a_tx = (uint32_t)(p.C / 8) * (STRIDE == 1 ? HALO_H * HALO_W * 16 : 4 * HALO_S2_W * HALO_S2_W * 16);
       int stg = 0;
       uint32_t par = 1;
       for (int mt = mt0; mt < m_tiles; mt += mt_step) {
@@ -336,9 +350,16 @@
         mbar_wait(empty_bar(stg), par);
         const uint32_t sa = sa0 + stg * a_stage;
         mbar_expect_tx(full_bar(stg), a_tx);
-        for (int cg = 0; cg < p.C / 8; ++cg)
-          tma_load_tiled_4d(sa + (uint32_t)cg * HALO_CG_BYTES, &map_a, full_bar(stg), 8 * cg, tw * HALO_TILE - 1, th * HALO_TILE - 1,
-                            n_img);
+        if (STRIDE == 1) {
+          for (int cg = 0; cg < p.C / 8; ++cg)
+            tma_load_tiled_4d(sa + (uint32_t)cg * HALO_CG_BYTES, &map_a, full_bar(stg), 8 * cg, tw * HALO_TILE - 1,
+                              th * HALO_TILE - 1, n_img);
+        } else {
+          for (int sg = 0; sg < 4; ++sg)
+            for (int cg = 0; cg < p.C / 8; ++cg)
+              tma_load_tiled_4d(sa + (uint32_t)sg * a_sub + (uint32_t)cg * HALO_S2_CG_BYTES, &map_a, full_bar(stg), 8 * cg,
+                                2 * tw * HALO_TILE - 1 + (sg & 1), 2 * th * HALO_TILE - 1 + (sg >> 1), n_img);
+        }
         if (++stg == p.stages) {
           stg = 0;
           par ^= 1;
@@ -356,14 +377,14 @@
       const uint32_t sa = sa0 + stg * a_stage;
       wgmma_fence();
       int t = off > 0 ? 0 : CENTRE_TAP;
-      uint32_t sa_t = sa + (uint32_t)((t / 3) * HALO_W + t % 3) * 16u, sb_t = sb + (uint32_t)(p.tap_b[t] * ksteps) * b_box;
+      uint32_t sa_t = sa + a_tap(t), sb_t = sb + (uint32_t)(p.tap_b[t] * ksteps) * b_box;
       for (int k = 0, ks = 0, nk = 8 * off + ksteps; k < nk; ++k) {
-        const uint64_t da = smem_desc_noswizzle(sa_t + (uint32_t)(2 * ks) * HALO_CG_BYTES, HALO_CG_BYTES, HALO_W * 16);
+        const uint64_t da = smem_desc_noswizzle(sa_t + (uint32_t)(2 * ks) * a_cg, a_cg, a_row);
         const uint64_t db = smem_desc(sb_t + (uint32_t)ks * b_box, 32, 16u, 256u);
         mma_kk<BN>(acc, da, db, k != 0);
         if (++ks == (t == CENTRE_TAP ? ksteps : off) && ++t < 9) {
           ks = 0;
-          sa_t = sa + (uint32_t)((t / 3) * HALO_W + t % 3) * 16u;
+          sa_t = sa + a_tap(t);
           sb_t = sb + (uint32_t)(p.tap_b[t] * ksteps) * b_box;
         }
       }
@@ -533,14 +554,16 @@
 
 constexpr uint32_t WH_A_BYTES = WPIX * 128;
 
-__host__ __device__ constexpr uint32_t wgrad_halo_stage_bytes(int nb) {
-  return (WH_A_BYTES + (uint32_t)(nb / 8) * HALO_CG_BYTES + 1023u) & ~1023u;
-}
-
-template <int NB, int NT>
+__host__ __device__ constexpr uint32_t wgrad_halo_stage_bytes(int nb, int stride = 1) {
+  return (WH_A_BYTES + halo_a_stage(nb, stride) + 1023u) & ~1023u;
+}
+
+template <int NB, int NT, int STRIDE>
 __device__ __forceinline__ void wgrad_halo_consume(const WParams& p, uint32_t ring, uint32_t bars, int t0, int t1, int tap0, int rb,
                                                    int ctile) {
-  constexpr uint32_t stage_bytes = wgrad_halo_stage_bytes(NB);
+  constexpr uint32_t stage_bytes = wgrad_halo_stage_bytes(NB, STRIDE);
+  constexpr uint32_t x_row = (STRIDE == 1 ? HALO_W : HALO_S2_W) * 16, x_cg = STRIDE == 1 ? HALO_CG_BYTES : HALO_S2_CG_BYTES;
+  constexpr uint32_t x_sub = (NB / 8) * HALO_S2_CG_BYTES;
   const int wq = (threadIdx.x >> 5) & 3, lane = threadIdx.x & 31;
   auto full_bar = [&](int s) { return bars + 8u * s; };
   auto empty_bar = [&](int s) { return bars + 8u * (MAX_STAGES + s); };
@@ -554,12 +577,14 @@
       wgmma_fence();
 #pragma unroll
       for (int t = 0; t < NT; ++t) {
-        const int tap = tap0 + t;
-        const uint32_t sx_t = sx + (uint32_t)((tap / 3) * HALO_W + tap % 3) * 16u;
+        const int tap = tap0 + t, dh = tap / 3, dw = tap % 3;
+        const uint32_t sx_t = STRIDE == 1 ? sx + (uint32_t)(dh * HALO_W + dw) * 16u
+                                          : sx + (uint32_t)(2 * (dh == 1) + (dw == 1)) * x_sub +
+                                                (uint32_t)((dh >> 1) * HALO_S2_W + (dw >> 1)) * 16u;
 #pragma unroll
         for (int j = 0; j < WPIX / 16; ++j) {
           const uint64_t da = smem_desc(sa + (uint32_t)j * 16u * 128u, 128, WPIX * 128, 8 * 128);
-          const uint64_t db = smem_desc_noswizzle(sx_t + (uint32_t)j * 2u * HALO_W * 16u, HALO_W * 16, HALO_CG_BYTES);
+          const uint64_t db = smem_desc_noswizzle(sx_t + (uint32_t)j * 2u * x_row, x_row, x_cg);
           mma_mn<NB>(acc[t], da, db, (mt != t0 || j != 0) ? 1u : 0u);
         }
       }
@@ -600,12 +625,12 @@
   }
 }
 
-template <int NB>
+template <int NB, int STRIDE>
 __global__ void __launch_bounds__(NUM_THREADS, 1)
 wgrad3x3_halo_kernel(const __grid_constant__ CUtensorMap map_dy, const __grid_constant__ CUtensorMap map_x, const WParams p) {
   extern __shared__ __align__(1024) unsigned char smem_raw[];
   const uint32_t smem_base = (smem_u32(smem_raw) + 1023u) & ~1023u;
-  constexpr uint32_t a_bytes = WH_A_BYTES, stage_bytes = wgrad_halo_stage_bytes(NB);
+  constexpr uint32_t a_bytes = WH_A_BYTES, stage_bytes = wgrad_halo_stage_bytes(NB, STRIDE);
   const uint32_t ctrl = smem_base + p.stages * stage_bytes;
   auto full_bar = [&](int s) { return ctrl + 8u * s; };
   auto empty_bar = [&](int s) { return ctrl + 8u * (MAX_STAGES + s); };
@@ -629,7 +654,7 @@
 
   if (warp == 0) {
     if (elect_one()) {
-      const uint32_t tx = a_bytes + (NB / 8) * (HALO_H * HALO_W * 16);
+      const uint32_t tx = a_bytes + (NB / 8) * (STRIDE == 1 ? HALO_H * HALO_W * 16 : 4 * HALO_S2_W * HALO_S2_W * 16);
       int stg = 0;
       uint32_t par = 1;
       for (int mt = t0; mt < t1; ++mt) {
@@ -640,9 +665,16 @@
         const uint32_t sa = smem_base + stg * stage_bytes;
         mbar_expect_tx(full_bar(stg), tx);
         tma_load_tiled_4d(sa, &map_dy, full_bar(stg), 64 * rb, tw * HALO_TILE, th * HALO_TILE, n_img);
-        for (int cg = 0; cg < NB / 8; ++cg)
-          tma_load_tiled_4d(sa + a_bytes + (uint32_t)cg * HALO_CG_BYTES, &map_x, full_bar(stg), ctile * NB + 8 * cg,
-                            tw * HALO_TILE - 1, th * HALO_TILE - 1, n_img);
+        if (STRIDE == 1) {
+          for (int cg = 0; cg < NB / 8; ++cg)
+            tma_load_tiled_4d(sa + a_bytes + (uint32_t)cg * HALO_CG_BYTES, &map_x, full_bar(stg), ctile * NB + 8 * cg,
+                              tw * HALO_TILE - 1, th * HALO_TILE - 1, n_img);
+        } else {
+          for (int sg = 0; sg < 4; ++sg)
+            for (int cg = 0; cg < NB / 8; ++cg)
+              tma_load_tiled_4d(sa + a_bytes + (uint32_t)(sg * (NB / 8) + cg) * HALO_S2_CG_BYTES, &map_x, full_bar(stg),
+                                ctile * NB + 8 * cg, 2 * tw * HALO_TILE - 1 + (sg & 1), 2 * th * HALO_TILE - 1 + (sg >> 1), n_img);
+        }
         if (++stg == p.stages) {
           stg = 0;
           par ^= 1;
@@ -653,13 +685,13 @@
     const int wg = (warp >> 2) - 1;
     const uint32_t ring = smem_base, bars = ctrl;
     if (!all_taps && wg == 0)
-      wgrad_halo_consume<NB, 1>(p, ring, bars, t0, t1, CENTRE_TAP, rb, ctile);
+      wgrad_halo_consume<NB, 1, STRIDE>(p, ring, bars, t0, t1, CENTRE_TAP, rb, ctile);
     else if (!all_taps)
-      wgrad_halo_consume<NB, 0>(p, ring, bars, t0, t1, 0, rb, ctile);
+      wgrad_halo_consume<NB, 0, STRIDE>(p, ring, bars, t0, t1, 0, rb, ctile);
     else if (wg == 0)
-      wgrad_halo_consume<NB, 5>(p, ring, bars, t0, t1, 0, rb, ctile);
+      wgrad_halo_consume<NB, 5, STRIDE>(p, ring, bars, t0, t1, 0, rb, ctile);
     else
-      wgrad_halo_consume<NB, 4>(p, ring, bars, t0, t1, 5, rb, ctile);
+      wgrad_halo_consume<NB, 4, STRIDE>(p, ring, bars, t0, t1, 5, rb, ctile);
   }
 }
 
@@ -674,12 +706,16 @@
 int g_num_sms = 0;
 long long g_launches = 0;
 long long g_halo_launches = 0;
+long long g_halo_s2_launches = 0;
 long long g_wgrad_halo_launches = 0;
+long long g_wgrad_halo_s2_launches = 0;
 bool g_force_im2col = false;
 bool g_wgrad_force_im2col = false;
 long long launch_count() { return g_launches; }
 long long halo_launch_count() { return g_halo_launches; }
+long long halo_s2_launch_count() { return g_halo_s2_launches; }
 long long wgrad_halo_launch_count() { return g_wgrad_halo_launches; }
+long long wgrad_halo_s2_launch_count() { return g_wgrad_halo_s2_launches; }
 void force_im2col(bool on) { g_force_im2col = on; }
 void wgrad_force_im2col(bool on) { g_wgrad_force_im2col = on; }
 
@@ -705,10 +741,10 @@
 }
 
 int encode_tiled(CUtensorMap* map, const void* ptr, int rank, const cuuint64_t* dims, const cuuint64_t* byte_strides,
-                 const cuuint32_t* box, CUtensorMapSwizzle swizzle, const char* what) {
-  const cuuint32_t elem_strides[5] = {1, 1, 1, 1, 1};
+                 const cuuint32_t* box, CUtensorMapSwizzle swizzle, const char* what, const cuuint32_t* elem_strides) {
+  const cuuint32_t unit_strides[5] = {1, 1, 1, 1, 1};
   const CUresult r = g_tiled(map, CU_TENSOR_MAP_DATA_TYPE_BFLOAT16, (cuuint32_t)rank, const_cast<void*>(ptr), dims, byte_strides, box,
-                             elem_strides, CU_TENSOR_MAP_INTERLEAVE_NONE, swizzle, CU_TENSOR_MAP_L2_PROMOTION_L2_128B,
+                             elem_strides ? elem_strides : unit_strides, CU_TENSOR_MAP_INTERLEAVE_NONE, swizzle, CU_TENSOR_MAP_L2_PROMOTION_L2_128B,
                              CU_TENSOR_MAP_FLOAT_OOB_FILL_NONE);
   if (r == CUDA_SUCCESS) return SGB_OK;
   char shape[256] = "";
@@ -739,9 +775,13 @@
   return SGB_E_CUDA;
 }
 
-int encode_halo_map(CUtensorMap* map, const void* x, int N, int H, int W, int C, int pitch) {
+int encode_halo_map(CUtensorMap* map, const void* x, int N, int H, int W, int C, int pitch, int stride = 1) {
   const cuuint64_t dims[4] = {(cuuint64_t)C, (cuuint64_t)W, (cuuint64_t)H, (cuuint64_t)N};
   const cuuint64_t strides[3] = {(cuuint64_t)pitch * 2, (cuuint64_t)W * pitch * 2, (cuuint64_t)H * W * pitch * 2};
+  if (stride == 2) {
+    const cuuint32_t box[4] = {8, 2 * HALO_S2_W - 1, 2 * HALO_S2_W - 1, 1}, estr[4] = {1, 2, 2, 1};
+    return encode_tiled(map, x, 4, dims, strides, box, CU_TENSOR_MAP_SWIZZLE_NONE, "stride-2 halo", estr);
+  }
   const cuuint32_t box[4] = {8, HALO_W, HALO_H, 1};
   return encode_tiled(map, x, 4, dims, strides, box, CU_TENSOR_MAP_SWIZZLE_NONE, "halo");
 }
@@ -790,12 +830,15 @@
                              {48, conv_wgmma_kernel<48, SKIP>}, {64, conv_wgmma_kernel<64, SKIP>},
                              {96, conv_wgmma_kernel<96, SKIP>}, {128, conv_wgmma_kernel<128, SKIP>}};
 template <bool SKIP>
-Variant<ConvFn> g_halo[6] = {{16, conv3x3_halo_kernel<16, SKIP>}, {32, conv3x3_halo_kernel<32, SKIP>},
-                             {48, conv3x3_halo_kernel<48, SKIP>}, {64, conv3x3_halo_kernel<64, SKIP>},
-                             {96, conv3x3_halo_kernel<96, SKIP>}, {128, conv3x3_halo_kernel<128, SKIP>}};
+Variant<ConvFn> g_halo[6] = {{16, conv3x3_halo_kernel<16, SKIP, 1>}, {32, conv3x3_halo_kernel<32, SKIP, 1>},
+                             {48, conv3x3_halo_kernel<48, SKIP, 1>}, {64, conv3x3_halo_kernel<64, SKIP, 1>},
+                             {96, conv3x3_halo_kernel<96, SKIP, 1>}, {128, conv3x3_halo_kernel<128, SKIP, 1>}};
+Variant<ConvFn> g_halo_s2[2] = {{48, conv3x3_halo_kernel<48, false, 2>}, {96, conv3x3_halo_kernel<96, false, 2>}};
 Variant<WgradFn> g_wgrad[6] = {{16, wgrad_wgmma_kernel<16>}, {32, wgrad_wgmma_kernel<32>}, {48, wgrad_wgmma_kernel<48>},
                                {64, wgrad_wgmma_kernel<64>}, {96, wgrad_wgmma_kernel<96>}, {128, wgrad_wgmma_kernel<128>}};
-Variant<WgradFn> g_wgrad_halo[3] = {{16, wgrad3x3_halo_kernel<16>}, {32, wgrad3x3_halo_kernel<32>}, {48, wgrad3x3_halo_kernel<48>}};
+template <int STRIDE>
+Variant<WgradFn> g_wgrad_halo[3] = {{16, wgrad3x3_halo_kernel<16, STRIDE>}, {32, wgrad3x3_halo_kernel<32, STRIDE>},
+                                    {48, wgrad3x3_halo_kernel<48, STRIDE>}};
 
 template <class Fn, int N>
 int prepare(Variant<Fn> (&table)[N], int bn, const char* what, Variant<Fn>*& var) {
@@ -826,9 +869,9 @@
   return best;
 }
 
-size_t halo_smem(int C, int bn, int n, bool stats, int stages) {
+size_t halo_smem(int C, int bn, int n, bool stats, int stages, int stride = 1) {
   const size_t b_bytes = ((size_t)9 * C * bn * 2 + 1023) & ~(size_t)1023;
-  const size_t a_stage = ((size_t)(C / 8) * HALO_CG_BYTES + 1023) & ~(size_t)1023;
+  const size_t a_stage = halo_a_stage(C, stride);
   return 1024 + b_bytes + (size_t)stages * a_stage + HALO_CTRL_BYTES + (stats ? (size_t)(8 * 2 * bn + 4 * n) * 4 : 0);
 }
 
@@ -850,6 +893,13 @@
   return 0;
 }
 
+int halo_s2_bn(const Problem& q) {
+  if (q.R != 3 || q.S != 3 || q.stride != 2 || q.pad != 1 || q.ntaps > 0 || q.out_mode != 0 || q.C > 48) return 0;
+  if (q.H != 2 * q.P || q.W != 2 * q.Q || q.P < 40 || q.Q < 40 || !halo_tiles_fit(q.P, q.Q)) return 0;
+  const int bn = pick_bn(q.b_rows);
+  return (bn == 48 || bn == 96) && halo_smem(q.C, bn, q.b_rows, q.stats != nullptr, 2, 2) <= 227 * 1024 ? bn : 0;
+}
+
 int launch_halo(const Problem& q, const Params& p0, int bn, cudaStream_t st) {
   Params p = p0;
   p.n_tiles = (p.N + bn - 1) / bn;
@@ -857,22 +907,26 @@
   p.halo_thw = p.halo_tw * ((q.P + HALO_TILE - 1) / HALO_TILE);
   p.M = q.N * p.halo_thw;
   p.centre_n = 0;
+  const int s = q.stride;
   Variant<ConvFn>* var = nullptr;
-  if (int rc = prepare(p.centre_c > 0 ? g_halo<true> : g_halo<false>, bn, "conv3x3_halo_kernel", var)) return rc;
+  const int rc = s == 2 ? prepare(g_halo_s2, bn, "conv3x3_halo_kernel", var)
+                        : prepare(p.centre_c > 0 ? g_halo<true> : g_halo<false>, bn, "conv3x3_halo_kernel", var);
+  if (rc) return rc;
   int ctas_per_sm = max_ctas_per_sm(var->regs);
   int stages = 0;
   for (;; --ctas_per_sm) {
     const size_t budget = (ctas_per_sm == 1 ? 227u : 227u / ctas_per_sm - 1u) * 1024u;
-    for (stages = HALO_MAX_STAGES; stages >= 2 && halo_smem(q.C, bn, p.N, p.stats != nullptr, stages) > budget; --stages) {
-    }
+    for (stages = HALO_MAX_STAGES; stages >= 2 && halo_smem(q.C, bn, p.N, p.stats != nullptr, stages, s) > budget; --stages) {
+    }
+    if (s == 2) stages &= ~1;
     if (stages >= 2 || ctas_per_sm == 1) break;
   }
   if (stages < 2) { sgb_set_error("conv3x3_halo: tile does not fit shared memory"); return SGB_E_UNSUPPORTED; }
   p.stages = stages;
-  const size_t smem = halo_smem(q.C, bn, p.N, p.stats != nullptr, stages);
+  const size_t smem = halo_smem(q.C, bn, p.N, p.stats != nullptr, stages, s);
 
   alignas(64) CUtensorMap map_a, map_b;
-  if (int rc = encode_halo_map(&map_a, q.a, q.N, q.H, q.W, q.C, q.a_pitch)) return rc;
+  if (int rc = encode_halo_map(&map_a, q.a, q.N, q.H, q.W, q.C, q.a_pitch, s)) return rc;
   const cuuint64_t b_dims[2] = {(cuuint64_t)q.b_cols, (cuuint64_t)q.b_rows}, b_strides[1] = {(cuuint64_t)q.b_cols * 2};
   const cuuint32_t b_box[2] = {16, (cuuint32_t)bn};
   if (int rc = encode_tiled(&map_b, q.b, 2, b_dims, b_strides, b_box, CU_TENSOR_MAP_SWIZZLE_32B, "halo B")) return rc;
@@ -881,7 +935,7 @@
   if (per_nt < 1) per_nt = 1;
   var->fn<<<per_nt * p.n_tiles, NUM_THREADS, smem, st>>>(map_a, map_b, p);
   ++g_launches;
-  ++g_halo_launches;
+  ++(s == 2 ? g_halo_s2_launches : g_halo_launches);
   return sgb_cuda_check(cudaGetLastError(), "conv3x3_halo_kernel");
 }
 
@@ -892,7 +946,8 @@
   p.N = q.b_rows;
   p.C = q.C;
   p.KC = q.C % 64 == 0 ? 64 : (q.C % 32 == 0 ? 32 : 16);
-  if (p.KC < 64 && q.C > 32) p.KC = 64;
+  const bool s2_dgrad_96 = q.out_mode == 1 && q.ntaps > 0 && q.C == 96;
+  if (p.KC < 64 && q.C > 32 && !s2_dgrad_96) p.KC = 64;
   const int bn = pick_bn(p.N);
   p.n_tiles = (p.N + bn - 1) / bn;
   p.P = q.P; p.Q = q.Q; p.stride = q.stride; p.pad = q.pad;
@@ -919,8 +974,10 @@
       return SGB_E_INVALID;
     (q.flip ? p.centre_c : p.centre_n) = q.centre_from;
   }
-  if (!g_force_im2col)
+  if (!g_force_im2col) {
     if (const int hbn = halo_bn(q)) return launch_halo(q, p, hbn, st);
+    if (const int hbn = halo_s2_bn(q)) return launch_halo(q, p, hbn, st);
+  }
   Variant<ConvFn>* var = nullptr;
   if (int rc = prepare(p.centre_n > 0 || p.centre_c > 0 ? g_conv<true> : g_conv<false>, bn, "conv_wgmma_kernel", var)) return rc;
   const uint32_t a_bytes = BLOCK_M * p.KC * 2, b_bytes = ((uint32_t)(bn * p.KC * 2) + 1023u) & ~1023u;
@@ -983,16 +1040,23 @@
   return q.C % 32 == 0 ? 32 : (q.C % 48 == 0 ? 48 : 16);
 }
 
+int wgrad_halo_s2_nb(const WgradProblem& q) {
+  if (q.R != 3 || q.S != 3 || q.stride != 2 || q.pad != 1 || q.H != 2 * q.P || q.W != 2 * q.Q || q.C > 48) return 0;
+  if (q.P < 40 || q.Q < 40 || !halo_tiles_fit(q.P, q.Q)) return 0;
+  return q.C == 48 ? 48 : 16;
+}
+
 int launch_wgrad_halo(const WgradProblem& q, const WParams& p0, int nb, cudaStream_t st) {
   WParams p = p0;
   p.n_ctiles = q.C / nb;
   p.halo_tw = (q.Q + HALO_TILE - 1) / HALO_TILE;
   p.halo_thw = p.halo_tw * ((q.P + HALO_TILE - 1) / HALO_TILE);
   p.tiles = q.N * p.halo_thw;
+  const int s = q.stride;
   Variant<WgradFn>* var = nullptr;
-  if (int rc = prepare(g_wgrad_halo, nb, "wgrad3x3_halo_kernel", var)) return rc;
+  if (int rc = prepare(s == 2 ? g_wgrad_halo<2> : g_wgrad_halo<1>, nb, "wgrad3x3_halo_kernel", var)) return rc;
   const int ctas_per_sm = max_ctas_per_sm(var->regs);
-  const uint32_t stage_bytes = wgrad_halo_stage_bytes(nb);
+  const uint32_t stage_bytes = wgrad_halo_stage_bytes(nb, s);
   const uint32_t budget = (ctas_per_sm == 1 ? 227u : 113u) * 1024u - 1024u - CTRL_BAR_BYTES;
   p.stages = (int)(budget / stage_bytes);
   if (p.stages > MAX_STAGES) p.stages = MAX_STAGES;
@@ -1008,10 +1072,10 @@
   const cuuint64_t dy_strides[3] = {(cuuint64_t)q.y_pitch * 2, (cuuint64_t)q.Q * q.y_pitch * 2, (cuuint64_t)q.P * q.Q * q.y_pitch * 2};
   const cuuint32_t dy_box[4] = {64, HALO_TILE, HALO_TILE, 1};
   if (int rc = encode_tiled(&map_dy, q.dy, 4, dy_dims, dy_strides, dy_box, CU_TENSOR_MAP_SWIZZLE_128B, "dy tile")) return rc;
-  if (int rc = encode_halo_map(&map_x, q.x, q.N, q.H, q.W, q.C, q.x_pitch)) return rc;
+  if (int rc = encode_halo_map(&map_x, q.x, q.N, q.H, q.W, q.C, q.x_pitch, s)) return rc;
   var->fn<<<splits * items, NUM_THREADS, smem, st>>>(map_dy, map_x, p);
   ++g_launches;
-  ++g_wgrad_halo_launches;
+  ++(s == 2 ? g_wgrad_halo_s2_launches : g_wgrad_halo_launches);
   return sgb_cuda_check(cudaGetLastError(), "wgrad3x3_halo_kernel");
 }
 
@@ -1034,8 +1098,10 @@
   for (int t = 0; t < q.R * q.S; ++t) p.items += (wgrad_row_blocks(p, t) + 1) / 2;
   p.cpad = q.C;
   p.dw = q.dw;
-  if (!g_wgrad_force_im2col)
+  if (!g_wgrad_force_im2col) {
     if (const int nb = wgrad_halo_nb(q)) return launch_wgrad_halo(q, p, nb, st);
+    if (const int nb = wgrad_halo_s2_nb(q)) return launch_wgrad_halo(q, p, nb, st);
+  }
   Variant<WgradFn>* var = nullptr;
   if (int rc = prepare(g_wgrad, nb, "wgrad_wgmma_kernel", var)) return rc;
   const uint32_t stage_bytes = 2 * WPIX * 128 + (uint32_t)(nb / p.CB) * WPIX * p.CB * 2;
diff --git a/super_gradients_b200/csrc/conv_sm100.h b/super_gradients_b200/csrc/conv_sm100.h
--- a/super_gradients_b200/csrc/conv_sm100.h
+++ b/super_gradients_b200/csrc/conv_sm100.h
@@ -15,8 +15,10 @@
 
 long long launch_count();
 long long halo_launch_count();
+long long halo_s2_launch_count();
 void force_im2col(bool on);
 long long wgrad_halo_launch_count();
+long long wgrad_halo_s2_launch_count();
 void wgrad_force_im2col(bool on);
 
 }
diff --git a/super_gradients_b200/csrc/sm100_host.h b/super_gradients_b200/csrc/sm100_host.h
--- a/super_gradients_b200/csrc/sm100_host.h
+++ b/super_gradients_b200/csrc/sm100_host.h
@@ -7,6 +7,6 @@
 int init_driver();
 
 int encode_tiled(CUtensorMap* map, const void* ptr, int rank, const cuuint64_t* dims, const cuuint64_t* byte_strides,
-                 const cuuint32_t* box, CUtensorMapSwizzle swizzle, const char* what);
+                 const cuuint32_t* box, CUtensorMapSwizzle swizzle, const char* what, const cuuint32_t* elem_strides = nullptr);
 
 }
diff --git a/super_gradients_b200/lib.py b/super_gradients_b200/lib.py
--- a/super_gradients_b200/lib.py
+++ b/super_gradients_b200/lib.py
@@ -156,8 +156,10 @@
     "sgb_check_device": (c_int, []),
     "sgb_sm100_launches": (c_int64, []),
     "sgb_conv_halo_launches": (c_int64, []),
+    "sgb_conv_halo_s2_launches": (c_int64, []),
     "sgb_conv_force_im2col": (None, [_I]),
     "sgb_conv_wgrad_halo_launches": (c_int64, []),
+    "sgb_conv_wgrad_halo_s2_launches": (c_int64, []),
     "sgb_conv_wgrad_force_im2col": (None, [_I]),
     "sgb_conv_fprop": (c_int, [POINTER(ConvDesc), P, P, P, POINTER(Epilogue), P]),
     "sgb_conv_dgrad": (c_int, [POINTER(ConvDesc), P, P, P, _I, P]),
@@ -245,7 +247,7 @@
 
 _lib = None
 
-LAUNCH_COUNT = {"sgb_tal_assign": 4, "sgb_lamb_step": 2, "sgb_clip_grad_norm": 2, "sgb_atss_assign": 3, "sgb_pose_tal_assign": 4, "sgb_sm100_launches": 0, "sgb_stem_recompute_launches": 0, "sgb_conv_halo_launches": 0, "sgb_conv_force_im2col": 0, "sgb_conv_wgrad_halo_launches": 0, "sgb_conv_wgrad_force_im2col": 0, "sgb_sliding_window_merge_workspace_bytes": 0, "sgb_sliding_window_merge_launches": 0, "sgb_last_error": 0, "sgb_version": 0, "sgb_check_device": 0}
+LAUNCH_COUNT = {"sgb_tal_assign": 4, "sgb_lamb_step": 2, "sgb_clip_grad_norm": 2, "sgb_atss_assign": 3, "sgb_pose_tal_assign": 4, "sgb_sm100_launches": 0, "sgb_stem_recompute_launches": 0, "sgb_conv_halo_launches": 0, "sgb_conv_halo_s2_launches": 0, "sgb_conv_force_im2col": 0, "sgb_conv_wgrad_halo_launches": 0, "sgb_conv_wgrad_halo_s2_launches": 0, "sgb_conv_wgrad_force_im2col": 0, "sgb_sliding_window_merge_workspace_bytes": 0, "sgb_sliding_window_merge_launches": 0, "sgb_last_error": 0, "sgb_version": 0, "sgb_check_device": 0}
 LAUNCHES = [0]
 
 
```

New measurement: 989.2, median of 6. No clear change (+0.2%).
